# VITA-Group/UVC

Measured on AMD Instinct MI355X. Metric: images/sec UVC Stage-1 step, DeiT-Tiny budget=0.5, higher is better.
Workload: dtype bf16; 1 GPU; deit_tiny_patch16_224 Stage-1 UVC-train step, budget 0.5, per-GPU batch 512, 224x224x3 synthetic, soft distillation alpha 0.1, block gating on; global_batch=512, parallelism=dp1

## Files before the change

### include/uvc_kernels.h

```cpp
#ifndef UVC_KERNELS_H
#define UVC_KERNELS_H
#include <stdint.h>
#ifdef __cplusplus
extern "C" {
#endif

enum { UVC_F32 = 0, UVC_BF16 = 1 };

enum {
  UVC_EPI_NONE = 0,
  UVC_EPI_BIAS = 1,
  UVC_EPI_BIAS_GELU = 2,
  UVC_EPI_BIAS_RESID = 3,
  UVC_EPI_BIAS_RESID_GATE = 4,
  UVC_EPI_DGELU = 5,
  UVC_EPI_BIAS_GELU_OUT = 6,
  UVC_EPI_BIAS_GELU_GRAD = 7,
  UVC_EPI_MUL_AUX = 8,
  UVC_EPI_BIAS_GELU_GRAD_Q8 = 9,
  UVC_EPI_MUL_AUX_Q8 = 10
};
#define UVC_Q8_LO (-0.13f)
#define UVC_Q8_STEP (1.26f / 255.0f)

// ... 41 lines not shown
  void* o;
  float* lse;
  const void* dout;
  void* dqkv;
  float* delta;
  int32_t B, N, H, head_dim, dtype;
  float scale;
  const int32_t* head_keep;
  int32_t variant;
  int32_t grid;
  int32_t v_dim;
} uvc_attn_args;
int uvc_attention_fwd(const uvc_attn_args* args, void* stream);
int uvc_attention_bwd(const uvc_attn_args* args, void* stream);
int uvc_attention_bwd_vdim(const uvc_attn_args* args, void* stream);

typedef struct uvc_qkv_attn_args {
  const void* h;
  const void* w;
  const float* bias;
  void* qkv;
  void* o;
  float* lse;
  int32_t B, N, H, D, dtype;
  float scale;
  int32_t grid;
} uvc_qkv_attn_args;
int uvc_qkv_attention_supported(int32_t B, int32_t N, int32_t H, int32_t D, int32_t dtype);
int uvc_qkv_attention_fwd(const uvc_qkv_attn_args* args, void* stream);

typedef struct uvc_attn_tok_args {
  const void* qkv;
  void* o;
  const void* dout;
  void* dqkv;
  int32_t B, N, H, head_dim, ntok, dtype;
  float scale;
  const int32_t* head_keep;
} uvc_attn_tok_args;
int uvc_attention_tok_fwd(const uvc_attn_tok_args* args, void* stream);
int uvc_attention_tok_bwd(const uvc_attn_tok_args* args, void* stream);

int uvc_copy_row_groups(const void* src, void* dst, int64_t groups, int64_t group_bytes, int64_t src_group_stride, int64_t dst_group_stride,
                        void* stream);

typedef struct uvc_ln_args {
  const void* x;
  const float* gamma; const float* beta;
  void* y; float* mean; float* rstd;
  const void* dy;
  void* dx;
  const void* add1; const float* a1;
  const void* add2; const float* a2;
  float* partial;
  float* dgamma; float* dbeta;
  float* dots;
  float eps, beta_acc;
  int32_t rows, D, rows_per_group, dtype, y_is_f32, dy_is_f32;
  int64_t group_stride;
  int32_t g_lowp;
  int32_t defer_reduce;
  int32_t x_lowp;
  int32_t reserved;
} uvc_ln_args;
typedef struct uvc_ln_reduce_item { const float* partial; float* dgamma; float* dbeta; float* dots; int32_t nblocks; int32_t reserved; } uvc_ln_reduce_item;
int uvc_layernorm_bwd_reduce_batch(const uvc_ln_reduce_item* items, int32_t n, int32_t D, float beta_acc, void* stream);
int uvc_layernorm_fwd(const uvc_ln_args* args, void* stream);
int uvc_layernorm_bwd(const uvc_ln_args* args, void* stream);
int uvc_layernorm_bwd_blocks(int32_t rows);
int uvc_layernorm_bwd_nblocks(int32_t rows);

typedef struct uvc_gemm_lnbwd_args {
  const void* A; const void* W;
  const void* x; const float* mean; const float* rstd; const float* gamma;
  const void* add1; const float* a1; const void* add2; const float* a2;
  void* dx; float* partial;
  int32_t M, D, K, dtype;
  int32_t variant;
  int32_t x_lowp;
} uvc_gemm_lnbwd_args;
int uvc_gemm_lnbwd_supported(int32_t M, int32_t D, int32_t K, int32_t dtype);
int uvc_gemm_lnbwd_nblocks(int32_t M);
int uvc_gemm_nt_lnbwd(const uvc_gemm_lnbwd_args* args, void* stream);

typedef struct uvc_mlp_args {
  const void* x; const float* gamma; const float* beta;
  const void* w1; const float* b1; const void* w2; const float* b2;
  void* out;
  int32_t M, D, F;
  float eps;
  const void* x_prev; const float* gate;
  void* h; float* mean; float* rstd; void* gp; void* u;
  const float* next_gamma; const float* next_beta; void* next_h; float* next_mean; float* next_rstd;
  int32_t rows_lowp;
  int32_t reserved;
} uvc_mlp_args;
int uvc_mlp_fused_supported(int32_t D, int32_t F, int32_t dtype);
int uvc_mlp_fused_fwd(const uvc_mlp_args* args, void* stream);

typedef struct uvc_loss_args {
  const float* o; const float* o_kd; const float* y_soft; const float* teacher;
  float* loss; float* d_o; float* d_okd; float* row_scratch;
  float alpha, tau;
  int32_t B, C, kind;
} uvc_loss_args;
int uvc_distill_loss(const uvc_loss_args* args, void* stream);

int uvc_grad_sqnorm(const float* g, int64_t n, float* partial , float* sq , int32_t accumulate, void* stream);
typedef struct uvc_adamw_args {
  float* p; const float* g; float* m; float* v;
  void* p_shadow;
  const float* sq;
  float* gnorm_out;
  int64_t n;
  float lr, beta1, beta2, eps, weight_decay, max_norm;
  int32_t step;
  const uint8_t* flags;
} uvc_adamw_args;
int uvc_adamw_step(const uvc_adamw_args* args, void* stream);
int uvc_scale_by_clip(float* g, int64_t n, const float* sq, float max_norm, void* stream);

int uvc_patchify(const float* x, void* out, int32_t B, int32_t C, int32_t S, int32_t P, int32_t dtype, void* stream);
int uvc_assemble_tokens(const float* pe, const float* cls, const float* dist, const float* pos, const float* row_mask,
                        void* tok, int32_t B, int32_t P, int32_t D, int32_t ntok, int32_t tok_lowp , void* stream);
int uvc_assemble_tokens_bwd(const void* dtok, const float* pe, const float* row_mask, void* dpe, float* dpos, float* dcls,
                            float* ddist, float* dmask, int32_t B, int32_t P, int32_t D, int32_t ntok, int32_t dtype,
                            int32_t dpe_is_f32, int32_t dtok_lowp, float beta_acc, void* stream);
int uvc_colsum(const void* X, int32_t M, int32_t N, int32_t ldx, int32_t dtype, int32_t x_is_f32, float* partial, float* out,
               float alpha, const float* alpha_ptr, float beta, const float* row_weight , void* stream);
int uvc_patch_gate_sigmoid(const float* pg, float* mask, int32_t B, int32_t P, int32_t hard, void* stream);
int uvc_patch_gate_sigmoid_bwd(const float* pg, const float* dmask, float* dpg, int32_t B, int32_t P, float beta_acc, void* stream);
int uvc_patch_scores(const float* pe, const float* w, const float* bias, float* scores, int32_t rows, int32_t D, void* stream);
int uvc_patch_topk_mask(const float* scores, const float* e, float* mask, float* ysoft, float* psoft, int32_t B, int32_t P, int32_t k,
                        float tau, void* stream);
int uvc_patch_topk_mask_bwd(const float* dmask, const float* ysoft, const float* psoft, float* dscores, int32_t B, int32_t P, float tau,
                            void* stream);
int uvc_add_outer(void* X, const float* row_weight, const float* w, int32_t rows, int32_t D, int32_t dtype, int32_t x_is_f32, void* stream);
int uvc_colsum_blocks(int32_t M);
int uvc_mixup_batch(float* x, int32_t B, int32_t C, int32_t H, int32_t W, float lam, float one_minus_lam, int32_t use_cutmix,
                    int32_t yl, int32_t yh, int32_t xl, int32_t xh, void* stream);
int uvc_mixup_target(const int64_t* labels, float* y, int32_t B, int32_t C, float lam, float one_minus_lam, float on_value,
                     float off_value, void* stream);
int uvc_mlp_gather_shadows(const float* W1, const float* b1, const float* W2, const int32_t* idx, int32_t D, int32_t F, int32_t width,
                           void* w1c, void* w1t, void* w2c, void* w2t, float* b1c, int32_t dtype, void* stream);
int uvc_mlp_scatter_grads(const float* dw1c, const float* dw2c, const float* db1c, const int32_t* inv, const float* b1, const float* db2,
                          int32_t D, int32_t F, int32_t width, float* dW1, float* dW2, float* db1, float beta_acc, int32_t dtype, void* stream);
int uvc_apply_masks(float* params, const float* mask, int64_t n, void* stream);
int uvc_cast_transpose(const float* W, int32_t R, int32_t C, void* w_bf16, void* wt, int32_t dtype, void* stream);
int uvc_cast_transpose_multi(const float* params, void* shadow, int32_t n, const int64_t* srcs, const int32_t* Rs, const int32_t* Cs,
                             const int64_t* ws, const int64_t* wts, int32_t dtype, void* stream);
int uvc_exp_noise(float* out, int64_t n, uint64_t seed, uint64_t step, uint32_t site, void* stream);

int uvc_gate_distrib(const float* g, const float* e, float* d, int32_t L, int32_t mode, float eps, void* stream);
int uvc_gate_grad(const float* g, const float* d, const float* dots, float* dg, int32_t L, int32_t mode, float eps,
                  float beta_acc, void* stream);

#ifdef __cplusplus
}
#endif
#endif
```

### include/uvc_vit.h

```cpp
#ifndef UVC_VIT_H
#define UVC_VIT_H
#include <stdint.h>
#ifdef __cplusplus
extern "C" {
#endif

#define UVC_VIT_MAX_DEPTH 32

typedef struct uvc_vit_cfg {
  int32_t img_size, patch_size, in_chans, num_classes, embed_dim, depth, num_heads, hidden;
  int32_t ntok;
  int32_t dtype;
  float ln_eps;
  int32_t no_qkv_bias;
  int32_t resid_f32;
  int32_t reserved;
} uvc_vit_cfg;

typedef struct uvc_vit_offsets {
  int64_t cls_token, dist_token, pos_embed, patch_w, patch_b;
  int64_t blk[UVC_VIT_MAX_DEPTH][12];
  int64_t norm_w, norm_b, head_w, head_b, headd_w, headd_b;
  int64_t n_main;
  int64_t gate;
  int64_t gumbel_w, gumbel_b;
  int64_t patch_gating;
  int64_t skip[UVC_VIT_MAX_DEPTH][2];
  int64_t n_total;
} uvc_vit_offsets;

typedef struct uvc_vit_shadow_offsets {
  int64_t patch_w;
  int64_t blk_w[UVC_VIT_MAX_DEPTH][4];
  int64_t blk_wt[UVC_VIT_MAX_DEPTH][4];
  int64_t head_w, head_wt, headd_w, headd_wt;
  int64_t n_total;
} uvc_vit_shadow_offsets;

int uvc_vit_layout(const uvc_vit_cfg* cfg, uvc_vit_offsets* off, uvc_vit_shadow_offsets* soff);
int64_t uvc_vit_workspace_bytes(const uvc_vit_cfg* cfg, int32_t batch, int32_t training);
int uvc_stream_create(int32_t priority_class, void** out);
int uvc_vit_ws_offsets(const uvc_vit_cfg* cfg, int32_t batch, int32_t training, int64_t* pe_off, int64_t* dpe_off);

int uvc_vit_update_shadows(const uvc_vit_cfg* cfg, const float* params, void* shadow, void* stream);

typedef struct uvc_mlp_compact {
  int32_t width; int32_t reserved;
  const void* w1; const void* w1t; const void* w2; const void* w2t; const float* b1;
  float* dw1; float* dw2; float* db1;
  const int32_t* inv;
} uvc_mlp_compact;

typedef struct uvc_vit_io {
  const float* params;
  void* shadow;
  float* grads;
  void* workspace; int64_t workspace_bytes;
  const float* x;
  float* logits;
  float* logits_dist;
  const float* d_logits;
  const float* d_logits_dist;
  const float* gate_d;
  const int32_t* run_block;
  const float* patch_mask;
  float* d_patch_mask;
  int32_t batch;
  int32_t training;
  int32_t gate_mode;
  float gate_eps;
  float accumulate;
  int32_t stage_begin, stage_end;
  void* side_stream;
  const uvc_mlp_compact* mlp_compact;
  const int32_t* head_keep;
  int32_t full_tail;
  int32_t fused_train_mlp;
  const void* patches_in;
  int32_t fuse_next_ln;
  int32_t force_generic;
  int32_t head_keep_bwd;
  int32_t shared_bwd_streams;
  int32_t gelu_grad_bf16;
} uvc_vit_io;

int uvc_vit_forward(const uvc_vit_cfg* cfg, const uvc_vit_io* io, void* stream);
int uvc_vit_backward(const uvc_vit_cfg* cfg, const uvc_vit_io* io, void* stream);

typedef struct uvc_compact_block { int32_t heads, v_dim, hidden, reserved; } uvc_compact_block;
int uvc_vit_compact_layout(const uvc_vit_cfg* cfg, const uvc_compact_block* blocks, int32_t nblocks, uvc_vit_offsets* off,
                           uvc_vit_shadow_offsets* soff);
int64_t uvc_vit_compact_workspace_bytes(const uvc_vit_cfg* cfg, const uvc_compact_block* blocks, int32_t nblocks, int32_t batch);
int uvc_vit_compact_update_shadows(const uvc_vit_cfg* cfg, const uvc_compact_block* blocks, int32_t nblocks, const float* params, void* shadow,
                                   void* stream);
int uvc_vit_compact_forward(const uvc_vit_cfg* cfg, const uvc_compact_block* blocks, int32_t nblocks, const uvc_vit_io* io, void* stream);

int uvc_vit_compact_train_layout(const uvc_vit_cfg* cfg, const uvc_compact_block* blocks, int32_t nblocks, uvc_vit_offsets* off,
                                 uvc_vit_shadow_offsets* soff);
int64_t uvc_vit_compact_train_workspace_bytes(const uvc_vit_cfg* cfg, const uvc_compact_block* blocks, int32_t nblocks, int32_t batch);
int uvc_vit_compact_train_update_shadows(const uvc_vit_cfg* cfg, const uvc_compact_block* blocks, int32_t nblocks, const float* params, void* shadow,
                                         void* stream);
int uvc_vit_compact_frozen_ranges(const uvc_vit_cfg* cfg, const uvc_compact_block* blocks, int32_t nblocks, int64_t* ranges, int32_t cap,
                                  int32_t* count);
int uvc_vit_compact_train_forward(const uvc_vit_cfg* cfg, const uvc_compact_block* blocks, int32_t nblocks, const uvc_vit_io* io, void* stream);
int uvc_vit_compact_backward(const uvc_vit_cfg* cfg, const uvc_compact_block* blocks, int32_t nblocks, const uvc_vit_io* io, void* stream);

#ifdef __cplusplus
}
#endif
#endif
```

### uvc_amd/_lib.py

```python
from __future__ import annotations

import ctypes as C
import os

import torch

_HERE = os.path.dirname(os.path.abspath(__file__))
LIB_PATH = os.path.join(_HERE, "libuvc_hip.so")


class UvcHipError(RuntimeError):
    pass


class uvc_dims(C.Structure):
    _fields_ = [("L", C.c_int32), ("H", C.c_int32), ("hd", C.c_int32), ("D", C.c_int32), ("F", C.c_int32)]


class uvc_hyper(C.Structure):
    _fields_ = [(n, C.c_float) for n in ("budget", "slr", "rlr", "glr", "ylr", "plr", "zlr", "sl2wd", "z_grad_clip",
                                         "gating_weight", "eps")] + \
               [(n, C.c_int32) for n in ("gating_interval", "use_gumbel", "enable_block_gating")]


class uvc_state(C.Structure):
    _fields_ = [("s", C.c_void_p), ("r", C.c_void_p), ("y", C.c_void_p), ("p", C.c_void_p), ("z", C.c_void_p),
                ("gate", C.c_void_p), ("gate_grad", C.c_void_p), ("gate_momentum", C.c_void_p),
                ("gate_gsum", C.c_void_p), ("gate_counters", C.c_void_p), ("total_macs", C.c_void_p),
                ("embed_macs", C.c_float), ("resource_ub", C.c_float),
                ("scores1", C.c_void_p), ("scores2", C.c_void_p), ("scores3", C.c_void_p),
                ("rank1", C.c_void_p), ("rankh", C.c_void_p), ("rank3", C.c_void_p), ("out", C.c_void_p)]


class uvc_gemm_nt_args(C.Structure):
    _fields_ = [(n, C.c_void_p) for n in ("A", "B", "C", "C2", "bias", "R", "R2", "aux", "gate", "alpha_ptr")] + \
               [("alpha", C.c_float)] + \
               [(n, C.c_int32) for n in ("M", "N", "K", "lda", "ldb", "ldc", "ldr", "ldaux", "dtype", "a_is_f32",
                                         "c_is_f32", "epilogue", "force_generic", "r_is_f32")] + \
               [("ln_eps", C.c_float)] + [(n, C.c_void_p) for n in ("ln_gamma", "ln_beta", "ln_out", "ln_mean", "ln_rstd")]


class uvc_gemm_tn_args(C.Structure):
    _fields_ = [("A", C.c_void_p), ("B", C.c_void_p), ("C", C.c_void_p), ("workspace", C.c_void_p),
                ("workspace_bytes", C.c_int64), ("alpha_ptr", C.c_void_p), ("colsum_out", C.c_void_p), ("alpha", C.c_float),
                ("beta", C.c_float)] + \
               [(n, C.c_int32) for n in ("M", "N1", "N2", "lda", "ldb", "ldc", "dtype", "a_is_f32", "variant")]


class uvc_attn_args(C.Structure):
    _fields_ = [(n, C.c_void_p) for n in ("qkv", "o", "lse", "dout", "dqkv", "delta")] + \
               [(n, C.c_int32) for n in ("B", "N", "H", "head_dim", "dtype")] + [("scale", C.c_float), ("head_keep", C.c_void_p),
                                                                                ("variant", C.c_int32), ("grid", C.c_int32),
                                                                                ("v_dim", C.c_int32)]


class uvc_compact_block(C.Structure):
    _fields_ = [(n, C.c_int32) for n in ("heads", "v_dim", "hidden", "reserved")]


class uvc_qkv_attn_args(C.Structure):
    _fields_ = [(n, C.c_void_p) for n in ("h", "w", "bias", "qkv", "o", "lse")] + \
               [(n, C.c_int32) for n in ("B", "N", "H", "D", "dtype")] + [("scale", C.c_float), ("grid", C.c_int32)]


class uvc_attn_tok_args(C.Structure):
    _fields_ = [(n, C.c_void_p) for n in ("qkv", "o", "dout", "dqkv")] + \
               [(n, C.c_int32) for n in ("B", "N", "H", "head_dim", "ntok", "dtype")] + [("scale", C.c_float), ("head_keep", C.c_void_p)]


class uvc_ln_reduce_item(C.Structure):
    _fields_ = [(n, C.c_void_p) for n in ("partial", "dgamma", "dbeta", "dots")] + [("nblocks", C.c_int32), ("reserved", C.c_int32)]


class uvc_ln_args(C.Structure):
    _fields_ = [(n, C.c_void_p) for n in ("x", "gamma", "beta", "y", "mean", "rstd", "dy", "dx", "add1", "a1", "add2",
                                          "a2", "partial", "dgamma", "dbeta", "dots")] + \
               [("eps", C.c_float), ("beta_acc", C.c_float)] + \
               [(n, C.c_int32) for n in ("rows", "D", "rows_per_group", "dtype", "y_is_f32", "dy_is_f32")] + \
               [("group_stride", C.c_int64), ("g_lowp", C.c_int32), ("defer_reduce", C.c_int32), ("x_lowp", C.c_int32), ("reserved", C.c_int32)]


class uvc_gemm_lnbwd_args(C.Structure):
    _fields_ = [(n, C.c_void_p) for n in ("A", "W", "x", "mean", "rstd", "gamma", "add1", "a1", "add2", "a2", "dx", "partial")] + \
               [(n, C.c_int32) for n in ("M", "D", "K", "dtype", "variant", "x_lowp")]


class uvc_mlp_args(C.Structure):
    _fields_ = [(n, C.c_void_p) for n in ("x", "gamma", "beta", "w1", "b1", "w2", "b2", "out")] + \
               [(n, C.c_int32) for n in ("M", "D", "F")] + [("eps", C.c_float)] + \
               [(n, C.c_void_p) for n in ("x_prev", "gate", "h", "mean", "rstd", "gp", "u",
                                          "next_gamma", "next_beta", "next_h", "next_mean", "next_rstd")] + \
               [("rows_lowp", C.c_int32), ("reserved", C.c_int32)]


class uvc_loss_args(C.Structure):
    _fields_ = [(n, C.c_void_p) for n in ("o", "o_kd", "y_soft", "teacher", "loss", "d_o", "d_okd", "row_scratch")] + \
               [("alpha", C.c_float), ("tau", C.c_float), ("B", C.c_int32), ("C", C.c_int32), ("kind", C.c_int32)]


class uvc_adamw_args(C.Structure):
    _fields_ = [(n, C.c_void_p) for n in ("p", "g", "m", "v", "p_shadow", "sq", "gnorm_out")] + [("n", C.c_int64)] + \
               [(n, C.c_float) for n in ("lr", "beta1", "beta2", "eps", "weight_decay", "max_norm")] + \
               [("step", C.c_int32), ("flags", C.c_void_p)]


class uvc_unfold_args(C.Structure):
    _fields_ = [("src", C.c_void_p)] + [(n, C.c_int64) for n in ("sb", "sc", "sh", "sw")] + \
               [(n, C.c_int32) for n in ("B", "C", "H", "W", "k", "s", "p", "ldo", "out_is_f32", "dtype")] + \
               [("gamma", C.c_void_p), ("beta", C.c_void_p), ("eps", C.c_float), ("out", C.c_void_p), ("mean", C.c_void_p),
                ("rstd", C.c_void_p), ("dy", C.c_void_p), ("dy_is_f32", C.c_int32), ("dxu", C.c_void_p), ("partial", C.c_void_p),
                ("dgamma", C.c_void_p), ("dbeta", C.c_void_p), ("beta_acc", C.c_float), ("dxu_tap_major", C.c_int32)]


class uvc_t2t_stage(C.Structure):
    _fields_ = [("src", C.c_void_p)] + [(n, C.c_int64) for n in ("sb", "sc", "sh", "sw")] + \
               [(n, C.c_int32) for n in ("B", "C", "H", "W", "k", "s", "p", "T", "dim", "dimp", "dtype", "training")] + \
               [("eps", C.c_float), ("beta", C.c_float), ("need_dx", C.c_int32), ("reserved", C.c_int32)] + \
               [(n, C.c_void_p) for n in ("norm1_w", "norm1_b", "kqv_b", "w", "proj_b", "norm2_w", "norm2_b", "fc1_b", "fc2_b",
                                          "g_norm1_w", "g_norm1_b", "g_kqv_w", "g_kqv_b", "g_proj_w", "g_proj_b", "g_norm2_w", "g_norm2_b", "g_fc1_w", "g_fc1_b",
                                          "g_fc2_w", "g_fc2_b",
                                          "kqv_w", "kqv_wt", "proj_w", "proj_wt", "fc1_w", "fc1_wt", "fc2_w", "fc2_wt",
                                          "xn", "mean1", "rstd1", "kqv", "part", "kptv", "att", "x1", "h", "mean2", "rstd2", "u", "gp", "out",
                                          "dout", "da", "dh", "dx1", "datt", "dkqv", "dkptv", "dxn", "ln2_partial", "ln1_partial", "dxu", "tn_ws")] + \
               [("tn_ws_bytes", C.c_int64)]


class uvc_performer_args(C.Structure):
    _fields_ = [(n, C.c_void_p) for n in ("kqv", "w", "part", "kptv", "att")] + [("att_is_f32", C.c_int32)] + \
               [(n, C.c_void_p) for n in ("datt", "dskip", "dkqv", "dkptv")] + \
               [(n, C.c_int32) for n in ("g_is_f32", "B", "T", "dtype")]


class uvc_image_desc(C.Structure):
    _fields_ = [("src_offset", C.c_int64)] + \
               [(n, C.c_int32) for n in ("src_h", "src_w", "resize_h", "resize_w", "win_y", "win_x", "flip", "kh", "kv", "span0", "span",
                                         "order")] + [("ws_offset", C.c_int64)]


class uvc_image_prep_args(C.Structure):
    _fields_ = [("src", C.c_void_p), ("src_bytes", C.c_int64), ("desc", C.c_void_p), ("workspace", C.c_void_p),
                ("workspace_bytes", C.c_int64), ("out", C.c_void_p), ("mean", C.c_float * 3), ("std", C.c_float * 3)] + \
               [(n, C.c_int32) for n in ("B", "S", "out_dtype", "filter")]


class uvc_image_crop_desc(C.Structure):
    _fields_ = [("src_offset", C.c_int64)] + \
               [(n, C.c_int32) for n in ("img_h", "img_w", "crop_y", "crop_x", "crop_h", "crop_w", "resize_h", "resize_w", "win_y", "win_x", "flip",
                                         "kh", "kv", "span0", "span", "order")] + [("ws_offset", C.c_int64)]


class uvc_image_prep_crops_args(C.Structure):
    _fields_ = uvc_image_prep_args._fields_


UVC_F32, UVC_BF16 = 0, 1
UVC_IMAGE_OUT_F32, UVC_IMAGE_OUT_U8 = 0, 1
UVC_IMAGE_FILTER_BILINEAR, UVC_IMAGE_FILTER_BICUBIC = 0, 1
EPI_NONE, EPI_BIAS, EPI_BIAS_GELU, EPI_BIAS_RESID, EPI_BIAS_RESID_GATE, EPI_DGELU, EPI_BIAS_GELU_OUT, EPI_BIAS_GELU_GRAD, EPI_MUL_AUX = range(9)
EPI_BIAS_GELU_GRAD_Q8, EPI_MUL_AUX_Q8 = 9, 10
Q8_LO, Q8_STEP = -0.13, 1.26 / 255.0

_lib = None
VP = C.c_void_p
I32, I64, F32 = C.c_int32, C.c_int64, C.c_float

_SIGNATURES = {
    "uvc_scores": [VP, VP, uvc_dims, VP, VP, VP, VP, VP],
    "uvc_rank": [VP, VP, VP, uvc_dims, VP, VP, VP, VP],
    "uvc_prox": [VP, VP, uvc_dims, VP, VP, VP, VP, VP, VP, VP, C.c_double, VP, VP, VP, VP, VP],
    "uvc_dual_step": [C.POINTER(uvc_state), uvc_dims, uvc_hyper, VP, VP, C.c_int32, C.c_int32, VP],
    "uvc_resource": [C.POINTER(uvc_state), uvc_dims, uvc_hyper, VP, C.c_int32, VP, VP],
    "uvc_write_masks": [VP, VP, VP, uvc_dims, VP, VP, VP, VP, VP, VP],
    "uvc_gemm_nt": [C.POINTER(uvc_gemm_nt_args), VP],
    "uvc_gemm_nt_ln_supported": [I32, I32, I32, I32, I32],
    "uvc_gemm_nt_q8_supported": [I32, I32, I32, I32],
    "uvc_gemm_tn": [C.POINTER(uvc_gemm_tn_args), VP],
    "uvc_gemm_tn_workspace_bytes": [I32, I32, I32, C.POINTER(I64), C.POINTER(I32)],
    "uvc_attention_fwd": [C.POINTER(uvc_attn_args), VP],
    "uvc_attention_bwd": [C.POINTER(uvc_attn_args), VP],
    "uvc_attention_bwd_vdim": [C.POINTER(uvc_attn_args), VP],
    "uvc_qkv_attention_supported": [I32, I32, I32, I32, I32],
    "uvc_qkv_attention_fwd": [C.POINTER(uvc_qkv_attn_args), VP],
    "uvc_attention_tok_fwd": [C.POINTER(uvc_attn_tok_args), VP],
    "uvc_attention_tok_bwd": [C.POINTER(uvc_attn_tok_args), VP],
    "uvc_copy_row_groups": [VP, VP, I64, I64, I64, I64, VP],
    "uvc_layernorm_fwd": [C.POINTER(uvc_ln_args), VP],
    "uvc_layernorm_bwd": [C.POINTER(uvc_ln_args), VP],
    "uvc_layernorm_bwd_blocks": [I32],
    "uvc_layernorm_bwd_nblocks": [I32],
    "uvc_layernorm_bwd_reduce_batch": [C.POINTER(uvc_ln_reduce_item), I32, I32, F32, VP],
    "uvc_gemm_lnbwd_supported": [I32, I32, I32, I32],
    "uvc_gemm_lnbwd_nblocks": [I32],
    "uvc_gemm_nt_lnbwd": [C.POINTER(uvc_gemm_lnbwd_args), VP],
    "uvc_distill_loss": [C.POINTER(uvc_loss_args), VP],
    "uvc_grad_sqnorm": [VP, I64, VP, VP, I32, VP],
    "uvc_adamw_step": [C.POINTER(uvc_adamw_args), VP],
    "uvc_scale_by_clip": [VP, I64, VP, F32, VP],
    "uvc_patchify": [VP, VP, I32, I32, I32, I32, I32, VP],
    "uvc_assemble_tokens": [VP, VP, VP, VP, VP, VP, I32, I32, I32, I32, I32, VP],
    "uvc_assemble_tokens_bwd": [VP, VP, VP, VP, VP, VP, VP, VP, I32, I32, I32, I32, I32, I32, I32, F32, VP],
    "uvc_colsum": [VP, I32, I32, I32, I32, I32, VP, VP, F32, VP, F32, VP, VP],
    "uvc_patch_gate_sigmoid": [VP, VP, I32, I32, I32, VP],
    "uvc_patch_gate_sigmoid_bwd": [VP, VP, VP, I32, I32, F32, VP],
    "uvc_patch_scores": [VP, VP, VP, VP, I32, I32, VP],
    "uvc_patch_topk_mask": [VP, VP, VP, VP, VP, I32, I32, I32, F32, VP],
    "uvc_patch_topk_mask_bwd": [VP, VP, VP, VP, I32, I32, F32, VP],
    "uvc_add_outer": [VP, VP, VP, I32, I32, I32, I32, VP],
    "uvc_colsum_blocks": [I32],
    "uvc_apply_masks": [VP, VP, I64, VP],
    "uvc_mlp_gather_shadows": [VP, VP, VP, VP, I32, I32, I32, VP, VP, VP, VP, VP, I32, VP],
    "uvc_mlp_scatter_grads": [VP, VP, VP, VP, VP, VP, I32, I32, I32, VP, VP, VP, F32, I32, VP],
    "uvc_mixup_batch": [VP, I32, I32, I32, I32, F32, F32, I32, I32, I32, I32, I32, VP],
    "uvc_mixup_target": [VP, VP, I32, I32, F32, F32, F32, F32, VP],
    "uvc_stream_create": [I32, C.POINTER(VP)],
    "uvc_mlp_fused_supported": [I32, I32, I32],
    "uvc_mlp_fused_fwd": [C.POINTER(uvc_mlp_args), VP],
    "uvc_cast_transpose": [VP, I32, I32, VP, VP, I32, VP],
    "uvc_cast_transpose_multi": [VP, VP, I32, VP, VP, VP, VP, VP, I32, VP],
    "uvc_exp_noise": [VP, I64, C.c_uint64, C.c_uint64, C.c_uint32, VP],
    "uvc_gate_distrib": [VP, VP, VP, I32, I32, F32, VP],
    "uvc_gate_grad": [VP, VP, VP, VP, I32, I32, F32, F32, VP],
    "uvc_image_prep_workspace": [VP, I32, I32, I64, C.POINTER(I64)],
    "uvc_image_prep_workspace_filter": [VP, I32, I32, I64, I32, C.POINTER(I64)],
    "uvc_image_prep": [C.POINTER(uvc_image_prep_args), VP],
    "uvc_image_prep_crops_workspace": [VP, I32, I32, I64, C.POINTER(I64)],
    "uvc_image_prep_crops_workspace_filter": [VP, I32, I32, I64, I32, C.POINTER(I64)],
    "uvc_image_prep_crops": [C.POINTER(uvc_image_prep_crops_args), VP],
    "uvc_unfold_ln_fwd": [C.POINTER(uvc_unfold_args), VP],
    "uvc_unfold_ln_bwd": [C.POINTER(uvc_unfold_args), VP],
    "uvc_unfold_bwd_blocks": [I32],
    "uvc_fold_tokens": [VP, I32, I32, I32, VP, I32, I32, I32, I32, I32, I32, I32, I32, I32, VP],
    "uvc_performer_splits": [I32, I32],
    "uvc_performer_fwd": [C.POINTER(uvc_performer_args), VP],
    "uvc_performer_bwd": [C.POINTER(uvc_performer_args), VP],
    "uvc_t2t_stage_forward": [C.POINTER(uvc_t2t_stage), VP],
    "uvc_t2t_stage_backward": [C.POINTER(uvc_t2t_stage), VP],
}


VIT_SYMBOLS = ["uvc_vit_layout", "uvc_vit_workspace_bytes", "uvc_vit_ws_offsets", "uvc_vit_update_shadows", "uvc_vit_forward",
               "uvc_vit_backward", "uvc_vit_compact_layout", "uvc_vit_compact_workspace_bytes", "uvc_vit_compact_update_shadows",
               "uvc_vit_compact_forward",
               "uvc_vit_compact_train_layout", "uvc_vit_compact_train_workspace_bytes", "uvc_vit_compact_train_update_shadows",
               "uvc_vit_compact_frozen_ranges", "uvc_vit_compact_train_forward", "uvc_vit_compact_backward"]


def side_stream(device, priority_class=None):
    import torch
    if priority_class is None:
        priority_class = int(os.environ.get("UVC_SIDE_PRIORITY", "0"))
    out = VP()
    with torch.cuda.device(device):
        check(lib().uvc_stream_create(priority_class, C.byref(out)), "uvc_stream_create")
    return torch.cuda.ExternalStream(out.value, device=device)


def exported_symbols():
    return list(_SIGNATURES) + ["uvc_last_error"] + VIT_SYMBOLS


def lib():
    global _lib
    if _lib is None:
        if not os.path.exists(LIB_PATH):
            raise UvcHipError(f"{LIB_PATH} not found: build it with `python -m uvc_amd.build` "
                              "(there is no CPU fallback for the product path)")
        _lib = C.CDLL(LIB_PATH)
        _lib.uvc_last_error.restype = C.c_char_p
        for name, args in _SIGNATURES.items():
            fn = getattr(_lib, name)
            fn.argtypes = args
            fn.restype = C.c_int
    return _lib


def check(rc: int, what: str):
# ... 17 lines not shown
```

### uvc_amd/csrc/gemm.hip

```cpp
#include <type_traits>
#include "common.h"
#include "../../include/uvc_kernels.h"

template <typename T> struct Mma;
template <> struct Mma<bf16_t> {
  static constexpr int CH = 8;
  static constexpr int KSTEP = 32;
  typedef bf16x8 Frag;
  static __device__ __forceinline__ f32x4 mma(const Frag& a, const Frag& b, f32x4 c) {
    return __builtin_amdgcn_mfma_f32_16x16x32_bf16(a, b, c, 0, 0, 0);
  }
};
template <> struct Mma<float> {
  static constexpr int CH = 4;
  static constexpr int KSTEP = 16;
  typedef f32x4 Frag;
  static __device__ __forceinline__ f32x4 mma(const Frag& a, const Frag& b, f32x4 c) {
#pragma unroll
    for (int j = 0; j < 4; ++j) c = __builtin_amdgcn_mfma_f32_16x16x4f32(a[j], b[j], c, 0, 0, 0);
    return c;
  }
};

template <typename TS, typename T> struct ChunkLoad;
// ... 990 lines not shown
  if (q8 && (p->force_generic == 1 || p->a_is_f32 || p->c_is_f32 || p->ln_out || !uvc_gemm_nt_q8_supported(p->M, p->N, p->K, p->dtype) ||
             (p->ldaux ? p->ldaux : p->ldc) % 8 || p->ldc % 8 || p->ldb != p->K))
    return uvc_set_error_msg(UVC_ERR_UNSUPPORTED, "uvc_gemm_nt: the one-byte GELU' epilogues need bf16 A / C, K = 192, N % 256 == 0, M >= 4096 (uvc_gemm_nt_q8_supported)");
  NtArgs a;
  a.A = p->A; a.B = p->B; a.C = p->C; a.C2 = p->C2; a.bias = p->bias; a.R = p->R; a.R2 = p->R2; a.aux = p->aux;
  a.dptr = p->gate; a.M = p->M; a.N = p->N; a.K = p->K; a.lda = p->lda; a.ldb = p->ldb; a.ldc = p->ldc;
  a.ldr = p->ldr ? p->ldr : p->ldc; a.ldaux = p->ldaux ? p->ldaux : p->ldc; a.alpha = p->alpha; a.alpha_ptr = p->alpha_ptr;
  a.ln_gamma = p->ln_gamma; a.ln_beta = p->ln_beta; a.ln_out = p->ln_out; a.ln_mean = p->ln_mean; a.ln_rstd = p->ln_rstd; a.ln_eps = p->ln_eps;
  a.no_dma = p->force_generic == 2;
  const bool generic = p->force_generic == 1;
  hipStream_t st = (hipStream_t)stream;
  if (p->ln_out) {
    if (!p->ln_gamma || !p->ln_beta || (p->ln_mean != nullptr) != (p->ln_rstd != nullptr))
      return uvc_set_error_msg(UVC_ERR_ARG, "uvc_gemm_nt: ln_out needs ln_gamma, ln_beta (and ln_mean, ln_rstd together)");
    if (p->N == 384) {
      if (!uvc_gemm_nt_ln_supported(p->M, p->N, p->K, p->dtype, e) || generic || p->a_is_f32 || p->c_is_f32 || p->alpha != 1.0f || p->alpha_ptr || !row384_fwd_ok(a, e))
        return uvc_set_error_msg(UVC_ERR_UNSUPPORTED, "uvc_gemm_nt: ln_out is not available for this problem (uvc_gemm_nt_ln_supported; N = 384: bf16 C and R only)");
      return launch_row384_fwd(a, e, st);
    }
    if (!uvc_gemm_nt_ln_supported(p->M, p->N, p->K, p->dtype, e) || generic || p->a_is_f32 || p->alpha != 1.0f || p->alpha_ptr ||
        a.ldb != a.K || !wsn16_dma_ok(a) || ((uintptr_t)p->ln_out & 7) != 0)
      return uvc_set_error_msg(UVC_ERR_UNSUPPORTED, "uvc_gemm_nt: ln_out is not available for this problem (uvc_gemm_nt_ln_supported)");
    if (p->M % 16 != 0 && (p->C == (const void*)p->R || p->C == (const void*)p->R2))
      return uvc_set_error_msg(UVC_ERR_ARG, "uvc_gemm_nt: with ln_out and M % 16 != 0 the last row tile is computed twice: C must not alias R / R2");
    if (p->K == 192) return p->c_is_f32 ? launch_wsn16_dma<UVC_EPI_BIAS_RESID, 6, true, 7, false>(a, st) : launch_wsn16_dma<UVC_EPI_BIAS_RESID, 6, true, 7, true>(a, st);
    return p->c_is_f32 ? launch_wsn<float>(a, e, st) : launch_wsn<bf16_t>(a, e, st);
  }
  if (p->dtype == UVC_F32) {
    if (!p->a_is_f32 || !p->c_is_f32) return uvc_set_error_msg(UVC_ERR_ARG, "uvc_gemm_nt: float32 mode needs float32 A and C");
    return launch_nt_epi<float, float, float>(a, e, st);
  }
  if (p->dtype != UVC_BF16) return uvc_set_error_msg(UVC_ERR_ARG, "uvc_gemm_nt: dtype must be UVC_F32 or UVC_BF16");
  {
    if (!p->force_generic && !p->a_is_f32 && e == UVC_EPI_BIAS_RESID && p->K == 192 && p->N == 192 && a.ldb == 192 &&
        p->M >= 4096 && p->M % 16 == 0 && p->alpha == 1.0f && !p->alpha_ptr && wsn16_dma_ok(a))
      return p->c_is_f32 ? launch_wsn16_dma<UVC_EPI_BIAS_RESID, 6, false, 7, false>(a, st) : launch_wsn16_dma<UVC_EPI_BIAS_RESID, 6, false, 7, true>(a, st);
  }
  const bool ws = !generic && ws_ok(a, p->c_is_f32 ? 4 : 8);
  if (q8 && !ws) return uvc_set_error_msg(UVC_ERR_UNSUPPORTED, "uvc_gemm_nt: the one-byte GELU' epilogues exist in the K = 192 streaming kernel only");
  if (!generic && ws384_ok(a, e, p->c_is_f32 ? 4 : 8, p->a_is_f32 != 0)) {
    if (!p->c_is_f32 && a.N % 128 == 0 && a.N >= 512 && p->force_generic != 5) return launch_ws384<bf16_t, 8>(a, e, st);
    return p->c_is_f32 ? launch_ws384<float>(a, e, st) : launch_ws384<bf16_t>(a, e, st);
  }
  if (!generic && wsn_ok(a, e, p->a_is_f32 != 0))
    return p->c_is_f32 ? launch_wsn<float>(a, e, st) : launch_wsn<bf16_t>(a, e, st);
  if ((p->force_generic >> 8) == 1) {
    if (!nt8p_takes(a, p->a_is_f32 != 0)) return uvc_set_error_msg(UVC_ERR_UNSUPPORTED, "uvc_gemm_nt: shape not taken by the 8-phase kernel");
    return p->c_is_f32 ? launch_nt8p_f32(a, e, p->force_generic & 255, st) : launch_nt8p_bf16(a, e, p->force_generic & 255, st);
  }
  const bool few_tiles_wide = !p->c_is_f32 && a.N % 256 == 0 && nt8p_takes(a, p->a_is_f32 != 0);
  if (!generic && !a.no_dma && !(p->force_generic == 3 && few_tiles_wide && a.N < 1792) &&
      nt256_takes(a, p->a_is_f32 != 0, p->force_generic == 3 || p->force_generic == 4))
    return p->c_is_f32 ? launch_nt256_f32(a, e, st) : launch_nt256_bf16(a, e, st);
  if (!generic && !a.no_dma && few_tiles_wide && (a.M >= 2048 || p->force_generic == 3))
    return launch_nt8p_bf16(a, e, 0, st);
  if (p->a_is_f32) {
    if ((p->lda % 8) != 0) return uvc_set_error_msg(UVC_ERR_ARG, "uvc_gemm_nt: lda");
    if (ws) return p->c_is_f32 ? launch_ws<float, float>(a, e, st) : launch_ws<float, bf16_t>(a, e, st);
    return p->c_is_f32 ? launch_nt_epi<float, bf16_t, float>(a, e, st) : launch_nt_epi<float, bf16_t, bf16_t>(a, e, st);
  }
  if (ws) return p->c_is_f32 ? launch_ws<bf16_t, float>(a, e, st) : launch_ws<bf16_t, bf16_t>(a, e, st);
  return p->c_is_f32 ? launch_nt_epi<bf16_t, bf16_t, float>(a, e, st) : launch_nt_epi<bf16_t, bf16_t, bf16_t>(a, e, st);
}

template <typename T> struct Raw4L;
template <> struct Raw4L<float> {
  typedef f32x4 V;
  static __device__ __forceinline__ V ld(const float* p) { return *reinterpret_cast<const f32x4*>(p); }
  static __device__ __forceinline__ V zero() { return f32x4{0.f, 0.f, 0.f, 0.f}; }
  static __device__ __forceinline__ f32x4 cvt(const V& r) { return r; }
};
template <> struct Raw4L<bf16_t> {
  typedef u32x2 V;
  static __device__ __forceinline__ V ld(const bf16_t* p) { return *reinterpret_cast<const u32x2*>(p); }
  static __device__ __forceinline__ V zero() { return u32x2{0u, 0u}; }
  static __device__ __forceinline__ f32x4 cvt(const V& r) {
    return f32x4{__uint_as_float(r[0] << 16), __uint_as_float(r[0] & 0xffff0000u), __uint_as_float(r[1] << 16), __uint_as_float(r[1] & 0xffff0000u)};
  }
};
struct LnbArgs {
  const void* A; const void* W; const void* x; const float* mean; const float* rstd; const float* gamma;
  const void* add1; const float* a1; const void* add2; const float* a2; void* dx; float* partial;
  int M, K, want_dots;
};

template <int KT, bool XLOW>
__global__ __launch_bounds__(768) void k_gemm_wsn_lnbwd(LnbArgs g) {
  typedef Resid<typename std::conditional<XLOW, bf16_t, float>::type> XS_;
  typedef bf16_t T;
  typedef Mma<T> MM;
  constexpr int K = KT * 32, NTH = 768, D = 192, NWV = 12;
  constexpr int ROWB = K * 2 + 32, CPR = K / 8;
  constexpr int NLD = (16 * CPR + NTH - 1) / NTH;
  extern __shared__ __attribute__((aligned(16))) char smem[];
  char* sA0 = smem;
  char* sA1 = smem + 16 * ROWB;
  float* sRed = reinterpret_cast<float*>(smem + 2 * 16 * ROWB);
  float* sGam = sRed + 2 * 16 * NWV * 2;
  const int tid = threadIdx.x, lane = tid & 63, w = tid >> 6, gq = lane >> 4, li = lane & 15;
  const T* __restrict__ A = reinterpret_cast<const T*>(g.A);
  const T* __restrict__ W = reinterpret_cast<const T*>(g.W);
  const T* __restrict__ add1 = reinterpret_cast<const T*>(g.add1);
  const T* __restrict__ add2 = reinterpret_cast<const T*>(g.add2);
  T* __restrict__ dx = reinterpret_cast<T*>(g.dx);
  const int ntiles = (g.M + 15) / 16;
  const int n = w * 16 + gq * 4;

  typename MM::Frag bf[KT];
#pragma unroll
  for (int ks = 0; ks < KT; ++ks)
    bf[ks] = __builtin_bit_cast(typename MM::Frag, *reinterpret_cast<const u32x4*>(W + (size_t)(w * 16 + li) * K + (ks * 4 + gq) * 8));
  if (tid < D) sGam[tid] = g.gamma[tid];
  const float a1 = g.a1 ? *g.a1 : 1.f, a2 = g.a2 ? *g.a2 : 1.f;
  f32x4 dgam = {0.f, 0.f, 0.f, 0.f}, dbet = {0.f, 0.f, 0.f, 0.f};
  float dotA = 0.f, dotB = 0.f;
  constexpr float invD = 1.0f / (float)D;

  u32x4 ra[NLD];
  unsigned aoff[NLD];
#pragma unroll
  for (int i = 0; i < NLD; ++i) { const int id = tid + NTH * i; aoff[i] = (unsigned)((id / CPR) * K + (id % CPR) * 8); }
  auto gload = [&](int tile) {
    const int m0 = tile * 16;
    const u32x4 z = {0u, 0u, 0u, 0u};
#pragma unroll
    for (int i = 0; i < NLD; ++i) {
      const int row = (tid + NTH * i) / CPR;
      ra[i] = (row < 16 && m0 + row < g.M) ? *reinterpret_cast<const u32x4*>(A + ((unsigned)(m0 * K) + aoff[i])) : z;
    }
  };
  auto lstore = [&](char* buf) {
#pragma unroll
    for (int i = 0; i < NLD; ++i) {
      const int id = tid + NTH * i, row = id / CPR, c = id % CPR;
      if (row < 16) *reinterpret_cast<u32x4*>(buf + row * ROWB + c * 16) = ra[i];
    }
  };

  int tile = blockIdx.x;
  if (tile < ntiles) {
    gload(tile);
    lstore(sA0);
  }
  __syncthreads();
  int par = 0;
  for (; tile < ntiles; tile += gridDim.x) {
    const int next = tile + gridDim.x;
    if (next < ntiles) gload(next);
    const int m = tile * 16 + li;
    const bool ok = m < g.M;
    const unsigned ro = (unsigned)(ok ? m : 0) * (unsigned)D + (unsigned)n;
    const f32x4 xv = XS_::f4(XS_::ld4(g.x, ro));
    u32x2 r1 = {0u, 0u}, r2 = {0u, 0u};
    if (add1) r1 = *reinterpret_cast<const u32x2*>(add1 + ro);
    if (add2) r2 = *reinterpret_cast<const u32x2*>(add2 + ro);
    const float mean = g.mean[ok ? m : 0], rstd = ok ? g.rstd[m] : 0.f;
    const char* buf = par ? sA1 : sA0;
    f32x4 c0 = {0.f, 0.f, 0.f, 0.f};
#pragma unroll
    for (int ks = 0; ks < KT; ++ks) {
      c0 = MM::mma(bf[ks], lds_frag<T>(buf + li * ROWB + (ks * 4 + gq) * 16), c0);
      if (KT > 18 && (ks % 6) == 5) __builtin_amdgcn_sched_barrier(0);
    }
    float* red = sRed + par * (16 * NWV * 2);
    {
      const f32x4 gam = *reinterpret_cast<const f32x4*>(sGam + n);
      float p1 = 0.f, p2 = 0.f;
#pragma unroll
      for (int e = 0; e < 4; ++e) {
        const float xh = (xv[e] - mean) * rstd;
        const float gy = c0[e] * gam[e];
        dgam[e] += c0[e] * xh;
        dbet[e] += c0[e];
        p1 += gy;
        p2 += gy * xh;
      }
      p1 = sum_rows4(p1);
      p2 = sum_rows4(p2);
      if (gq == 0) *reinterpret_cast<f32x2*>(red + (li * NWV + w) * 2) = f32x2{p1, p2};
    }
    if (next < ntiles) lstore(par ? sA0 : sA1);
    __syncthreads();
    float c1 = 0.f, c2 = 0.f;
#pragma unroll
    for (int q = 0; q < NWV / 2; ++q) {
      const f32x4 t = *reinterpret_cast<const f32x4*>(red + li * NWV * 2 + q * 4);
      c1 += t[0]; c2 += t[1]; c1 += t[2]; c2 += t[3];
    }
    c1 *= invD; c2 *= invD;
    if (ok) {
      const f32x4 gam = *reinterpret_cast<const f32x4*>(sGam + n);
      const f32x4 v1 = {__uint_as_float(r1[0] << 16), __uint_as_float(r1[0] & 0xffff0000u), __uint_as_float(r1[1] << 16), __uint_as_float(r1[1] & 0xffff0000u)};
      const f32x4 v2 = {__uint_as_float(r2[0] << 16), __uint_as_float(r2[0] & 0xffff0000u), __uint_as_float(r2[1] << 16), __uint_as_float(r2[1] & 0xffff0000u)};
      float o[4];
#pragma unroll
      for (int e = 0; e < 4; ++e) {
        const float xh = (xv[e] - mean) * rstd;
        o[e] = rstd * (c0[e] * gam[e] - c1 - xh * c2);
        if (add1) o[e] += a1 * v1[e];
        if (add2) { o[e] += a2 * v2[e]; dotB += v2[e] * xv[e]; }
        dotA += o[e] * xv[e];
      }
      u32x2 q; q[0] = pack_bf16x2(o[0], o[1]); q[1] = pack_bf16x2(o[2], o[3]);
      *reinterpret_cast<u32x2*>(dx + ro) = q;
    }
    par ^= 1;
  }
#pragma unroll
  for (int e = 0; e < 4; ++e) {
#pragma unroll
    for (int o = 1; o < 16; o <<= 1) { dgam[e] += __shfl_xor(dgam[e], o, 64); dbet[e] += __shfl_xor(dbet[e], o, 64); }
  }
  float* P = g.partial + (size_t)blockIdx.x * (2 * D + 2);
  if (li == 0) {
    *reinterpret_cast<f32x2*>(P + n) = f32x2{dgam[0], dgam[1]}; *reinterpret_cast<f32x2*>(P + n + 2) = f32x2{dgam[2], dgam[3]};
    *reinterpret_cast<f32x2*>(P + D + n) = f32x2{dbet[0], dbet[1]}; *reinterpret_cast<f32x2*>(P + D + n + 2) = f32x2{dbet[2], dbet[3]};
  }
  dotA = wave_sum(dotA); dotB = wave_sum(dotB);
  __syncthreads();
  if (lane == 0) { sRed[2 * w] = dotA; sRed[2 * w + 1] = dotB; }
  __syncthreads();
  if (tid < 2) {
    float t = 0.f;
#pragma unroll
    for (int q = 0; q < NWV; ++q) t += sRed[2 * q + tid];
    P[2 * D + tid] = t;
  }
}

__device__ __forceinline__ unsigned lds_addr(const void* p) { return (unsigned)(size_t)(LDS_PTR(char))(char*)p; }
__device__ __forceinline__ u32x4 ds_read128_asm(unsigned addr, int off) {
  u32x4 v;
  asm volatile("ds_read_b128 %0, %1 offset:%2" : "=v"(v) : "v"(addr), "n"(off));
  return v;
}
template <int OFF> __device__ __forceinline__ u32x4 ds_read128(unsigned addr) {
  u32x4 v;
  asm volatile("ds_read_b128 %0, %1 offset:%2" : "=v"(v) : "v"(addr), "n"(OFF));
  return v;
}
__device__ __forceinline__ u32x2 ds_read64_a(unsigned addr) { u32x2 v; asm volatile("ds_read_b64 %0, %1" : "=v"(v) : "v"(addr)); return v; }
__device__ __forceinline__ float ds_read32_a(unsigned addr) { float v; asm volatile("ds_read_b32 %0, %1" : "=v"(v) : "v"(addr)); return v; }
__device__ __forceinline__ void ds_write64_a(unsigned addr, f32x2 v) { asm volatile("ds_write_b64 %0, %1" ::"v"(addr), "v"(v) : "memory"); }
template <int N> __device__ __forceinline__ void wait_lgkm() { asm volatile("s_waitcnt lgkmcnt(%0)" ::"n"(N) : "memory"); }
template <int N> __device__ __forceinline__ void wait_vm() { asm volatile("s_waitcnt vmcnt(%0)" ::"n"(N) : "memory"); }
#define TIE4(a, b, c, d) asm volatile("" : "+v"(a), "+v"(b), "+v"(c), "+v"(d))

template <int KT, bool HAS2, bool XLOW>
__global__ __launch_bounds__(768) void k_gemm_wsn_lnbwd_dma(LnbArgs g) {
  typedef bf16_t T;
  typedef Mma<T> MM;
  constexpr int K = KT * 32, D = 192, NWV = 12;
  constexpr int ROWB = K * 2 + 32, SA = ROWB / 16;
  constexpr int NA = (16 * SA + 63) / 64;
  constexpr int XSZ = XLOW ? 2 : 4, XSL = D * XSZ / 16;
  constexpr int XS = XSL + 2, XB = XS * 16, NX = (16 * XS + 63) / 64;
  constexpr int PS = 26, PB = PS * 16, NP = (16 * PS + 63) / 64;
  constexpr int I_X = NA, I_1 = I_X + NX, I_2 = I_1 + NP, NI = I_2 + NP;
  constexpr int STAGE = NI * 1024;
  static_assert((16 * SA) % 64 == 32, "spare half block behind the A image");
  constexpr int MR_OFF = (NA - 1) * 1024 + 512;
  static_assert(NI <= 5 * NWV && 3 * STAGE + 2 * 16 * NWV * 8 + D * 4 <= 160 * 1024, "ring does not fit");
  extern __shared__ __attribute__((aligned(16))) char smem[];
  float* sRed = reinterpret_cast<float*>(smem + 3 * STAGE);
  const int tid = threadIdx.x, lane = tid & 63, gq = lane >> 4, li = lane & 15;
  const int w = __builtin_amdgcn_readfirstlane(tid >> 6);
  const T* __restrict__ W = reinterpret_cast<const T*>(g.W);
  T* __restrict__ dx = reinterpret_cast<T*>(g.dx);
  const int ntiles = g.M / 16;
  const int n = w * 16 + gq * 4;

  typename MM::Frag bf[KT];
#pragma unroll
  for (int ks = 0; ks < KT; ++ks)
    bf[ks] = __builtin_bit_cast(typename MM::Frag, *reinterpret_cast<const u32x4*>(W + (size_t)(w * 16 + li) * K + (ks * 4 + gq) * 8));
  float* sGam = sRed + 2 * 16 * NWV * 2;
  if (tid < D) sGam[tid] = g.gamma[tid];
  const unsigned gaddr = lds_addr(sGam) + (unsigned)n * 4u;
  const float a1 = g.a1 ? *g.a1 : 1.f, a2 = g.a2 ? *g.a2 : 1.f;
  const bool has1 = g.add1 != nullptr;
  constexpr bool has2 = HAS2;
  f32x4 dgam = {0.f, 0.f, 0.f, 0.f}, dbet = {0.f, 0.f, 0.f, 0.f};
  float dotA = 0.f, dotB = 0.f;
  constexpr float invD = 1.0f / (float)D;

  const char* rb[5]; unsigned rstride[5], rdst[5], loff[5];
#pragma unroll
  for (int q = 0; q < 5; ++q) {
    int I = q * NWV + w;
    const bool dup = I >= NI || (I >= I_1 && I < I_2 && !has1) || (I >= I_2 && !has2);
    if (dup) I = w;
    const int sl = (I - (I < I_X ? 0 : I < I_1 ? I_X : I < I_2 ? I_1 : I_2)) * 64 + lane;
    rdst[q] = (unsigned)I * 1024u;
    if (I < I_X) {
      const int row = sl / SA, c = sl % SA;
      rb[q] = reinterpret_cast<const char*>(g.A); rstride[q] = 16u * K * 2u;
      loff[q] = row < 16 ? (unsigned)(row * K * 2 + (c < K / 8 ? c : 0) * 16) : 0u;
    } else if (I < I_1) {
      const int row = sl / XS, c = sl % XS;
      rb[q] = reinterpret_cast<const char*>(g.x); rstride[q] = 16u * D * (unsigned)XSZ;
      loff[q] = row < 16 ? (unsigned)(row * D * XSZ + (c < XSL ? c : 0) * 16) : 0u;
    } else {
      const int row = sl / PS, c = sl % PS;
      rb[q] = reinterpret_cast<const char*>(I < I_2 ? g.add1 : g.add2); rstride[q] = 16u * D * 2u;
      loff[q] = row < 16 ? (unsigned)(row * D * 2 + (c < 24 ? c : 0) * 16) : 0u;
    }
  }
  const long long mr_delta = reinterpret_cast<const char*>(g.rstd) - reinterpret_cast<const char*>(g.mean);
  const unsigned mr_lo = (unsigned)(lane & 3) * 16u;
  const bool mr_lane = lane >= 32 && lane < 40, mr_r = lane >= 36;
  auto issue_q = [&](int tile, int st, int q) {
    const int t = tile < ntiles ? tile : ntiles - 1;
    if (q < 5) {
      const char* src = rb[q] + ((unsigned long long)(unsigned)t * (unsigned long long)rstride[q] + (unsigned long long)loff[q]);
      char* dst = smem + st * STAGE + rdst[q];
      __builtin_amdgcn_global_load_lds((const void __attribute__((address_space(1)))*)src, (void __attribute__((address_space(3)))*)dst, 16, 0, 0);
    } else if (mr_lane) {
      const char* src = reinterpret_cast<const char*>(g.mean) + ((unsigned long long)(unsigned)t * 64ull + mr_lo) + (mr_r ? mr_delta : 0ll);
      char* dst = smem + st * STAGE + (NA - 1) * 1024;
      __builtin_amdgcn_global_load_lds((const void __attribute__((address_space(1)))*)src, (void __attribute__((address_space(3)))*)dst, 16, 0, 0);
    }
  };
  auto issue = [&](int tile, int st) {
#pragma unroll
    for (int q = 0; q < 6; ++q) issue_q(tile, st, q);
  };
  const unsigned s0 = lds_addr(smem);
  const unsigned fragoff = (unsigned)(li * ROWB + gq * 16);
  const unsigned xoff = (unsigned)(I_X * 1024 + li * XB + n * XSZ), poff = (unsigned)(I_1 * 1024 + li * PB + n * 2), moff = (unsigned)(MR_OFF + li * 4);
  const unsigned redr = lds_addr(sRed) + (unsigned)(li * NWV * 8);

  int tile = blockIdx.x;
  issue(tile, 0);
  issue(tile + gridDim.x, 1);
  wait_vm<6>();
  __builtin_amdgcn_s_barrier();
  int st = 0, par = 0;
  for (; tile < ntiles; tile += gridDim.x) {
    const int nt_ = tile + 2 * (int)gridDim.x, ns_ = st == 0 ? 2 : st - 1;
    const unsigned sb = s0 + (unsigned)(st * STAGE);
    f32x4 c0 = {0.f, 0.f, 0.f, 0.f};
    constexpr bool DB = KT <= 18;
    u32x4 fa[2], fb[2];
    const unsigned fr = sb + fragoff;
#define RD2(dst, ks0) dst[0] = ds_read128<(ks0) * 64>(fr); dst[1] = ds_read128<(ks0) * 64 + 64>(fr);
#define GROUP(gk, cur, nxt) if ((gk) < KT / 2) { \
      if (DB) { if ((gk) + 1 < KT / 2) { RD2(nxt, ((gk) + 1) * 2) wait_lgkm<2>(); } else wait_lgkm<0>(); \
                asm volatile("" : "+v"(cur[0]), "+v"(cur[1])); \
                c0 = MM::mma(bf[(gk) * 2], __builtin_bit_cast(typename MM::Frag, cur[0]), c0); \
                c0 = MM::mma(bf[(gk) * 2 + 1], __builtin_bit_cast(typename MM::Frag, cur[1]), c0); } \
      else if (((gk) & 1) == 0) { RD2(fa, (gk) * 2) RD2(fb, (gk) * 2 + 2) wait_lgkm<0>();  \
             asm volatile("" : "+v"(fa[0]), "+v"(fa[1]), "+v"(fb[0]), "+v"(fb[1])); \
             c0 = MM::mma(bf[(gk) * 2], __builtin_bit_cast(typename MM::Frag, fa[0]), c0); \
             c0 = MM::mma(bf[(gk) * 2 + 1], __builtin_bit_cast(typename MM::Frag, fa[1]), c0); \
             c0 = MM::mma(bf[(gk) * 2 + 2], __builtin_bit_cast(typename MM::Frag, fb[0]), c0); \
             c0 = MM::mma(bf[(gk) * 2 + 3], __builtin_bit_cast(typename MM::Frag, fb[1]), c0); } }
    static_assert(KT % 2 == 0 && KT <= 24, "pairs of k-steps");
    if (DB) { RD2(fa, 0) }
    GROUP(0, fa, fb) issue_q(nt_, ns_, 0); GROUP(1, fb, fa) GROUP(2, fa, fb) issue_q(nt_, ns_, 1); GROUP(3, fb, fa)
    GROUP(4, fa, fb) issue_q(nt_, ns_, 2); GROUP(5, fb, fa) GROUP(6, fa, fb) issue_q(nt_, ns_, 3); GROUP(7, fb, fa)
    GROUP(8, fa, fb) issue_q(nt_, ns_, 4); issue_q(nt_, ns_, 5); GROUP(9, fb, fa) GROUP(10, fa, fb) GROUP(11, fb, fa)
#undef GROUP
#undef RD2
    typename Resid<typename std::conditional<XLOW, bf16_t, float>::type>::Raw4 xr;
    if constexpr (XLOW) asm volatile("ds_read_b64 %0, %1" : "=v"(xr) : "v"(sb + xoff));
    else xr = ds_read128<0>(sb + xoff);
    u32x2 r1 = {0u, 0u}, r2 = {0u, 0u};
    if (has1) asm volatile("ds_read_b64 %0, %1" : "=v"(r1) : "v"(sb + poff));
    if (has2) asm volatile("ds_read_b64 %0, %1 offset:%2" : "=v"(r2) : "v"(sb + poff), "n"((I_2 - I_1) * 1024));
    float mean, rstd;
    asm volatile("ds_read_b32 %0, %1" : "=v"(mean) : "v"(sb + moff));
    asm volatile("ds_read_b32 %0, %1 offset:64" : "=v"(rstd) : "v"(sb + moff));
    u32x4 gr = ds_read128<0>(gaddr);
    wait_lgkm<0>();
    asm volatile("" : "+v"(xr), "+v"(r1), "+v"(r2), "+v"(mean), "+v"(rstd), "+v"(gr));
    const f32x4 xv = Resid<typename std::conditional<XLOW, bf16_t, float>::type>::f4(xr);
    f32x4 gam = __builtin_bit_cast(f32x4, gr);
    {
      float p1 = 0.f, p2 = 0.f;
#pragma unroll
      for (int e = 0; e < 4; ++e) {
        const float xh = (xv[e] - mean) * rstd;
        const float gy = c0[e] * gam[e];
        dgam[e] += c0[e] * xh;
        dbet[e] += c0[e];
        p1 += gy;
        p2 += gy * xh;
      }
      p1 = sum_rows4(p1);
      p2 = sum_rows4(p2);
      if (gq == 0) ds_write64_a(redr + (unsigned)(par * 16 * NWV * 8 + w * 8), f32x2{p1, p2});
#pragma unroll
      for (int e = 0; e < 4; ++e) c0[e] *= gam[e];
    }
    wait_vm<6>();
    wait_lgkm<0>();
    __builtin_amdgcn_s_barrier();
    float c1 = 0.f, c2 = 0.f;
    {
      const unsigned rr = redr + (unsigned)(par * 16 * NWV * 8);
      u32x4 t0 = ds_read128<0>(rr), t1 = ds_read128<16>(rr), t2 = ds_read128<32>(rr);
      wait_lgkm<0>();
      asm volatile("" : "+v"(t0), "+v"(t1), "+v"(t2));
      {
        const f32x4 a = __builtin_bit_cast(f32x4, t0), b = __builtin_bit_cast(f32x4, t1), c = __builtin_bit_cast(f32x4, t2);
        c1 += a[0]; c2 += a[1]; c1 += a[2]; c2 += a[3]; c1 += b[0]; c2 += b[1]; c1 += b[2]; c2 += b[3]; c1 += c[0]; c2 += c[1]; c1 += c[2]; c2 += c[3];
      }
      t0 = ds_read128<48>(rr); t1 = ds_read128<64>(rr); t2 = ds_read128<80>(rr);
      wait_lgkm<0>();
      asm volatile("" : "+v"(t0), "+v"(t1), "+v"(t2));
      {
        const f32x4 a = __builtin_bit_cast(f32x4, t0), b = __builtin_bit_cast(f32x4, t1), c = __builtin_bit_cast(f32x4, t2);
        c1 += a[0]; c2 += a[1]; c1 += a[2]; c2 += a[3]; c1 += b[0]; c2 += b[1]; c1 += b[2]; c2 += b[3]; c1 += c[0]; c2 += c[1]; c1 += c[2]; c2 += c[3];
      }
    }
    c1 *= invD; c2 *= invD;
    {
      const f32x4 v1 = {__uint_as_float(r1[0] << 16), __uint_as_float(r1[0] & 0xffff0000u), __uint_as_float(r1[1] << 16), __uint_as_float(r1[1] & 0xffff0000u)};
      const f32x4 v2 = {__uint_as_float(r2[0] << 16), __uint_as_float(r2[0] & 0xffff0000u), __uint_as_float(r2[1] << 16), __uint_as_float(r2[1] & 0xffff0000u)};
      float o[4];
#pragma unroll
      for (int e = 0; e < 4; ++e) {
        const float xh = (xv[e] - mean) * rstd;
        o[e] = rstd * (c0[e] - c1 - xh * c2);
        if (has1) o[e] += a1 * v1[e];
        if (has2) { o[e] += a2 * v2[e]; dotB += v2[e] * xv[e]; }
        dotA += o[e] * xv[e];
      }
      u32x2 q; q[0] = pack_bf16x2(o[0], o[1]); q[1] = pack_bf16x2(o[2], o[3]);
      *reinterpret_cast<u32x2*>(dx + ((size_t)(tile * 16 + li) * D + n)) = q;
    }
    st = st == 2 ? 0 : st + 1;
    par ^= 1;
  }
  wait_vm<0>();
  __syncthreads();
#pragma unroll
  for (int e = 0; e < 4; ++e) {
#pragma unroll
    for (int o = 1; o < 16; o <<= 1) { dgam[e] += __shfl_xor(dgam[e], o, 64); dbet[e] += __shfl_xor(dbet[e], o, 64); }
  }
  float* P = g.partial + (size_t)blockIdx.x * (2 * D + 2);
  if (li == 0) {
    *reinterpret_cast<f32x2*>(P + n) = f32x2{dgam[0], dgam[1]}; *reinterpret_cast<f32x2*>(P + n + 2) = f32x2{dgam[2], dgam[3]};
    *reinterpret_cast<f32x2*>(P + D + n) = f32x2{dbet[0], dbet[1]}; *reinterpret_cast<f32x2*>(P + D + n + 2) = f32x2{dbet[2], dbet[3]};
  }
  dotA = wave_sum(dotA); dotB = wave_sum(dotB);
  if (lane == 0) { sRed[2 * w] = dotA; sRed[2 * w + 1] = dotB; }
  __syncthreads();
  if (tid < 2) {
    float t = 0.f;
#pragma unroll
    for (int q = 0; q < NWV; ++q) t += sRed[2 * q + tid];
    P[2 * D + tid] = t;
  }
}
#undef TIE4

template <int EPI, int KT, bool LN, int NST, bool RLOW>
__global__ __launch_bounds__(768) void k_gemm_wsn16_dma(NtArgs g) {
  typedef bf16_t T;
  typedef Mma<T> MM;
  constexpr int K = KT * 32, D = 192, NWV = 12;
  constexpr int ROWB = K * 2 + 32, SA = ROWB / 16;
  constexpr int NA = (16 * SA + 63) / 64;
  constexpr int RSZ = RLOW ? 2 : 4, RSL = D * RSZ / 16;
  constexpr int XS = RSL + 2, XB = XS * 16, NX = (16 * XS + 63) / 64;
  constexpr bool GATE = EPI == UVC_EPI_BIAS_RESID_GATE;
  constexpr int I_R = NA, I_R2 = I_R + NX, NI = I_R2 + (GATE ? NX : 0);
  constexpr int STAGE = NI * 1024;
  constexpr int NPW = (NI + NWV - 1) / NWV;
  constexpr int LN_BYTES = LN ? 2 * 16 * NWV * 8 + 3 * D * 4 : 0;
  static_assert(NST >= 3 && NPW <= 5 && NST * STAGE + LN_BYTES <= 160 * 1024, "ring does not fit");
  extern __shared__ __attribute__((aligned(16))) char smem[];
  const int tid = threadIdx.x, lane = tid & 63, gq = lane >> 4, li = lane & 15;
  const int w = __builtin_amdgcn_readfirstlane(tid >> 6);
  const T* __restrict__ W = reinterpret_cast<const T*>(g.B);
  char* __restrict__ C = reinterpret_cast<char*>(g.C);
  const int ntiles = (g.M + 15) / 16;
  const int n = w * 16 + gq * 4;
  float* const sRed = reinterpret_cast<float*>(smem + NST * STAGE);
  float* const sGB = sRed + 2 * 16 * NWV * 2;
  if (LN) {
    if (tid < D) { sGB[tid] = g.ln_gamma[tid]; sGB[D + tid] = g.ln_beta[tid]; sGB[2 * D + tid] = g.bias[tid]; }
  }
  const unsigned gaddr = lds_addr(sGB) + (unsigned)n * 4u;
  const unsigned redr = lds_addr(sRed) + (unsigned)(li * NWV * 8);
  typename MM::Frag bf[KT];
#pragma unroll
  for (int ks = 0; ks < KT; ++ks)
    bf[ks] = __builtin_bit_cast(typename MM::Frag, *reinterpret_cast<const u32x4*>(W + (size_t)(w * 16 + li) * K + (ks * 4 + gq) * 8));
  float alpha = g.alpha;
  if (g.alpha_ptr) alpha *= *g.alpha_ptr;
  float d0 = 0.f, d1 = 1.f;
  if (GATE) { d0 = g.dptr[0]; d1 = g.dptr[1]; }
  f32x4 bias4 = {0.f, 0.f, 0.f, 0.f};
  if (!LN) bias4 = *reinterpret_cast<const f32x4*>(g.bias + n);

  const char* rb[NPW]; unsigned rstride[NPW], rdst[NPW], loff[NPW];
#pragma unroll
  for (int q = 0; q < NPW; ++q) {
    int I = q * NWV + w;
    if (I >= NI) I = w;
    const int sl = (I - (I < I_R ? 0 : I < I_R2 ? I_R : I_R2)) * 64 + lane;
    rdst[q] = (unsigned)I * 1024u;
    if (I < I_R) {
      const int row = sl / SA, c = sl % SA;
      rb[q] = reinterpret_cast<const char*>(g.A); rstride[q] = K * 2u;
      loff[q] = row < 16 ? (unsigned)(row * K * 2 + (c < K / 8 ? c : 0) * 16) : 0u;
    } else {
      const int row = sl / XS, c = sl % XS;
      rb[q] = reinterpret_cast<const char*>(I < I_R2 ? g.R : g.R2); rstride[q] = (unsigned)(D * RSZ);
      loff[q] = row < 16 ? (unsigned)(row * D * RSZ + (c < RSL ? c : 0) * 16) : 0u;
    }
  }
  auto issue = [&](int tile, int st) {
    const int t = tile < ntiles ? tile : ntiles - 1;
    const unsigned r0 = (unsigned)min(t * 16, g.M - 16);
#pragma unroll
    for (int q = 0; q < NPW; ++q) {
      const char* src = rb[q] + ((unsigned long long)r0 * (unsigned long long)rstride[q] + (unsigned long long)loff[q]);
      char* dst = smem + st * STAGE + rdst[q];
      __builtin_amdgcn_global_load_lds((const void __attribute__((address_space(1)))*)src, (void __attribute__((address_space(3)))*)dst, 16, 0, 0);
    }
  };
  const unsigned s0 = lds_addr(smem);
  const unsigned fragoff = (unsigned)(li * ROWB + gq * 16), roff = (unsigned)(I_R * 1024 + li * XB + n * RSZ);

// ... 96 lines not shown
      __builtin_amdgcn_s_barrier();
      const f32x4 r = RS::f4(rr), r2 = RS::f4(rr2);
      float o[4];
#pragma unroll
      for (int e = 0; e < 4; ++e) {
        o[e] = epi_scale_bias(c0[e], alpha, bias4[e]);
        o[e] += r[e];
        if (GATE) o[e] = epi_gate_mix(o[e], r2[e], d0, d1);
      }
      char* cp = C + ((size_t)(min(tile * 16, g.M - 16) + li) * g.ldc + n) * RSZ;
      if constexpr (RLOW) { u32x2 q; q[0] = pack_bf16x2(o[0], o[1]); q[1] = pack_bf16x2(o[2], o[3]); *reinterpret_cast<u32x2*>(cp) = q; }
      else *reinterpret_cast<f32x4*>(cp) = f32x4{o[0], o[1], o[2], o[3]};
    } else {
      u32x4 bq = ds_read128<2 * D * 4>(gaddr);
      wait_lgkm<0>();
      asm volatile("" : "+v"(rr), "+v"(rr2), "+v"(bq));
      const f32x4 r = RS::f4(rr), r2 = RS::f4(rr2), bv = __builtin_bit_cast(f32x4, bq);
      float o[4];
#pragma unroll
      for (int e = 0; e < 4; ++e) {
        o[e] = epi_scale_bias(c0[e], alpha, bv[e]);
        o[e] += r[e];
        if (GATE) o[e] = epi_gate_mix(o[e], r2[e], d0, d1);
      }
      u32x2 oq = {0u, 0u};
      if constexpr (RLOW) {
        oq[0] = pack_bf16x2(o[0], o[1]); oq[1] = pack_bf16x2(o[2], o[3]);
        const f32x4 t = Resid<bf16_t>::f4(oq);
#pragma unroll
        for (int e = 0; e < 4; ++e) o[e] = t[e];
      }
      {
        const float sm = sum_rows4((o[0] + o[1]) + (o[2] + o[3]));
        const float mw = sm * (1.0f / 16.0f);
        float qw = 0.f;
#pragma unroll
        for (int e = 0; e < 4; ++e) { const float dd = o[e] - mw; qw += dd * dd; }
        qw = sum_rows4(qw);
        if (gq == 0) ds_write64_a(redr + (unsigned)(par * 16 * NWV * 8 + w * 8), f32x2{mw, qw});
      }
      prow0 = min(tile * 16, g.M - 16);
      if constexpr (RLOW) *reinterpret_cast<u32x2*>(C + (size_t)prow0 * g.ldc * RSZ + (unsigned)((li * g.ldc + n) * RSZ)) = oq;
      else *reinterpret_cast<f32x4*>(C + (size_t)prow0 * g.ldc * RSZ + (unsigned)((li * g.ldc + n) * RSZ)) = f32x4{o[0], o[1], o[2], o[3]};
#pragma unroll
      for (int e = 0; e < 4; ++e) po[e] = o[e];
      have_prev = true;
      wait_vm<(NST - 2) * NPW>();
      wait_lgkm<0>();
      __builtin_amdgcn_s_barrier();
      par ^= 1;
    }
    st = st == NST - 1 ? 0 : st + 1;
  }
  if (LN && have_prev) {
    ln_issue(std::integral_constant<int, 0>{});
    wait_lgkm<0>(); ln_first();
    ln_issue(std::integral_constant<int, 32>{});
    wait_lgkm<0>(); ln_acc();
    ln_issue(std::integral_constant<int, 64>{}); lgr = ds_read128<0>(gaddr); lbr = ds_read128<D * 4>(gaddr);
    wait_lgkm<0>(); ln_acc(); ln_finish();
  }
  wait_vm<0>();
}

int launch_row384_lnbwd(const LnbArgs& a, int x_lowp, hipStream_t st);

extern "C" int uvc_gemm_lnbwd_supported(int32_t M, int32_t D, int32_t K, int32_t dtype) {
  if (dtype != UVC_BF16 || M < 4096) return 0;
  if (D == 192) return K == 768 || K == 576;
  return D == 384 && K % 64 == 0 && K >= 128 && (int64_t)M * K < (1ll << 30);
}
extern "C" int uvc_gemm_lnbwd_nblocks(int32_t M) { const int nt = ceil_div(M, 16); return nt < 256 ? nt : 256; }

extern "C" int uvc_gemm_nt_lnbwd(const uvc_gemm_lnbwd_args* p, void* stream) {
  if (!p || !p->A || !p->W || !p->x || !p->mean || !p->rstd || !p->gamma || !p->dx || !p->partial)
    return uvc_set_error_msg(UVC_ERR_ARG, "uvc_gemm_nt_lnbwd: null pointer");
  if (!uvc_gemm_lnbwd_supported(p->M, p->D, p->K, p->dtype))
    return uvc_set_error_msg(UVC_ERR_UNSUPPORTED, "uvc_gemm_nt_lnbwd: bf16, M >= 4096, D = 192 with K in {576, 768} or D = 384 with K % 64 == 0");
  if ((((uintptr_t)p->A | (uintptr_t)p->W | (uintptr_t)p->x | (uintptr_t)p->gamma) & 15) != 0 ||
      (((uintptr_t)p->add1 | (uintptr_t)p->add2 | (uintptr_t)p->dx | (uintptr_t)p->partial) & 7) != 0)
    return uvc_set_error_msg(UVC_ERR_ARG, "uvc_gemm_nt_lnbwd: misaligned buffer");
  LnbArgs a;
  a.A = p->A; a.W = p->W; a.x = p->x; a.mean = p->mean; a.rstd = p->rstd; a.gamma = p->gamma; a.add1 = p->add1; a.a1 = p->a1;
  a.add2 = p->add2; a.a2 = p->a2; a.dx = p->dx; a.partial = p->partial; a.M = p->M; a.K = p->K; a.want_dots = 1;
  const int grid = uvc_gemm_lnbwd_nblocks(p->M);
  hipStream_t st = (hipStream_t)stream;
  if (p->D == 384) return launch_row384_lnbwd(a, p->x_lowp, st);
#define LNB_LAUNCH(KT_) { \
    const size_t sh = (size_t)2 * 16 * (KT_ * 64 + 32) + (2 * 16 * 12 * 2 + 192) * sizeof(float); \
    if (p->x_lowp) { UVC_MAX_LDS(sh, k_gemm_wsn_lnbwd<KT_, true>); k_gemm_wsn_lnbwd<KT_, true><<<grid, 768, sh, st>>>(a); } \
    else { UVC_MAX_LDS(sh, k_gemm_wsn_lnbwd<KT_, false>); k_gemm_wsn_lnbwd<KT_, false><<<grid, 768, sh, st>>>(a); } }
  const bool use_dma = p->variant != 1;
  const bool al16 = (((uintptr_t)p->add1 | (uintptr_t)p->add2 | (uintptr_t)p->mean | (uintptr_t)p->rstd) & 15) == 0;
#define LNB_DMA_ONE(KT_, H2_, XL_) { UVC_MAX_LDS(sh, k_gemm_wsn_lnbwd_dma<KT_, H2_, XL_>); k_gemm_wsn_lnbwd_dma<KT_, H2_, XL_><<<grid, 768, sh, st>>>(a); }
#define LNB_LAUNCH_DMA(KT_) { \
    constexpr int NA_ = (16 * (KT_ * 4 + 2) + 63) / 64; \
    const int NI_ = NA_ + (p->x_lowp ? 7 : 13) + 7 + 7; \
    const size_t sh = (size_t)3 * NI_ * 1024 + (2 * 16 * 12 * 2 + 192) * sizeof(float); \
    if (p->x_lowp) { if (p->add2) LNB_DMA_ONE(KT_, true, true) else LNB_DMA_ONE(KT_, false, true) } \
    else { if (p->add2) LNB_DMA_ONE(KT_, true, false) else LNB_DMA_ONE(KT_, false, false) } }
  if (use_dma && al16 && p->M % 16 == 0) { if (p->K == 768) LNB_LAUNCH_DMA(24) else LNB_LAUNCH_DMA(18) }
  else if (p->K == 768) LNB_LAUNCH(24) else LNB_LAUNCH(18)
#undef LNB_LAUNCH_DMA
#undef LNB_DMA_ONE
#undef LNB_LAUNCH
  UVC_CHECK_LAUNCH();
  return UVC_OK;
}

#define NT_EPILOGUE_TILE(NH, MROW0, NCOL0, PD1, PD2)                                                                                 \
  {                                                                                                                           \
    constexpr bool PRE_ = sizeof(TC) == 2 && EpiOperands<EPI>::COUNT > 0;                                                     \
    constexpr int PD_ = EpiOperands<EPI>::COUNT >= 2 ? (PD2) : (PD1);                                                              \
    EpiPre<2> pre_[PD_];                                                                                                      \
    if constexpr (PRE_) {                                                                                                     \
      _Pragma("unroll") for (int h = 0; h < PD_ && h < (NH); ++h) nt_epilogue_prefetch<EPI, 16>(g, lane, (MROW0) + h * 16, (NCOL0), pre_[h]); \
    }                                                                                                                         \
    _Pragma("unroll") for (int h = 0; h < (NH); ++h) {                                                                        \
      _Pragma("unroll") for (int j = 0; j < 4; ++j)                                                                           \
        *reinterpret_cast<f32x4*>(stg_at<true>(stg, lane & 15, j * 4 + (lane >> 4))) = acc[h][j];                            \
      __builtin_amdgcn_wave_barrier();                                                                                        \
      nt_epilogue_rows<T, TC, EPI, 16, true, PRE_>(g, stg, lane, (MROW0) + h * 16, (NCOL0), alpha, d0, d1, bias_v, &pre_[h % PD_]); \
      if constexpr (PRE_) { if (h + PD_ < (NH)) nt_epilogue_prefetch<EPI, 16>(g, lane, (MROW0) + (h + PD_) * 16, (NCOL0), pre_[h % PD_]); } \
      __builtin_amdgcn_wave_barrier();                                                                                        \
    }                                                                                                                         \
  }

constexpr int G2_BM = 256, G2_BN = 256, G2_BK = 64;
constexpr int G2_OPB = 256 * 128;
constexpr int G2_STAGE = 2 * G2_OPB;
constexpr int G2_EPI = 8 * 16 * 64 * 4;
constexpr int G2_LDS = 2 * G2_STAGE + G2_EPI;

struct G2Frags { u32x4 a[8]; u32x4 b[4]; };

__device__ __forceinline__ bool g2_tile(int v, int tiles_m, int tiles_n, int& bm, int& bn) {
  const int xcd = v & 7, q = v >> 3;
  bn = q % tiles_n; bm = (q / tiles_n) * 8 + xcd;
  return bm < tiles_m;
}

template <typename TC, int EPI>
__global__ __launch_bounds__(512, 2) void k_gemm_nt256(NtArgs g, int tiles_m, int tiles_n, int nvirt) {
  typedef bf16_t T;
  typedef Mma<T> MM;
  extern __shared__ __attribute__((aligned(16))) char smem[];
  const int tid = threadIdx.x, lane = tid & 63;
  const int w = __builtin_amdgcn_readfirstlane(tid >> 6);
  const int wm = w >> 2, wn = w & 3;

  const __amdgpu_buffer_rsrc_t rA = __builtin_amdgcn_make_buffer_rsrc(const_cast<void*>(g.A), 0, (int)(((size_t)(g.M - 1) * g.lda + g.K) * 2), 0x00020000);
  const __amdgpu_buffer_rsrc_t rB = __builtin_amdgcn_make_buffer_rsrc(const_cast<void*>(g.B), 0, (int)(((size_t)(g.N - 1) * g.ldb + g.K) * 2), 0x00020000);
  const int lrow = lane >> 3, lchunk = (lane & 7) ^ lrow;
  const unsigned laneA = (unsigned)(((w * 8 + lrow) * g.lda + lchunk * 8) * 2), laneB = (unsigned)(((w * 8 + lrow) * g.ldb + lchunk * 8) * 2);
  const unsigned stepA = (unsigned)(64 * g.lda * 2), stepB = (unsigned)(64 * g.ldb * 2);
  auto issue1 = [&](int t, unsigned voA, unsigned voB, int kt, int st) {
    char* base = smem + st * G2_STAGE + w * 1024;
    const unsigned kb = (unsigned)(kt * G2_BK * 2);
    if (t < 4) __builtin_amdgcn_raw_ptr_buffer_load_lds(rA, (__attribute__((address_space(3))) void*)(base + t * 8192), 16, laneA + (voA + kb + t * stepA), 0, 0, 0);
    else __builtin_amdgcn_raw_ptr_buffer_load_lds(rB, (__attribute__((address_space(3))) void*)(base + G2_OPB + (t - 4) * 8192), 16, laneB + (voB + kb + (t - 4) * stepB), 0, 0, 0);
  };
  const unsigned s0 = lds_addr(smem);
  const unsigned sw0 = (unsigned)((((lane >> 4)) ^ (lane & 7)) * 16);
  const unsigned fa0 = s0 + (unsigned)((wm * 128 + (lane & 15)) * 128) + sw0;
  const unsigned fb0 = s0 + (unsigned)(G2_OPB + (wn * 64 + (lane & 15)) * 128) + sw0;
  auto rdfrags = [&](G2Frags& F, int st, int ks) {
    const unsigned a = (fa0 ^ (unsigned)(ks * 64)) + (unsigned)(st * G2_STAGE), b = (fb0 ^ (unsigned)(ks * 64)) + (unsigned)(st * G2_STAGE);
    F.b[0] = ds_read128<0 * 2048>(b); F.b[1] = ds_read128<1 * 2048>(b); F.b[2] = ds_read128<2 * 2048>(b); F.b[3] = ds_read128<3 * 2048>(b);
    F.a[0] = ds_read128<0 * 2048>(a); F.a[1] = ds_read128<1 * 2048>(a); F.a[2] = ds_read128<2 * 2048>(a); F.a[3] = ds_read128<3 * 2048>(a);
    F.a[4] = ds_read128<4 * 2048>(a); F.a[5] = ds_read128<5 * 2048>(a); F.a[6] = ds_read128<6 * 2048>(a); F.a[7] = ds_read128<7 * 2048>(a);
  };
  auto tie = [&](G2Frags& F) {
    asm volatile("" : "+v"(F.a[0]), "+v"(F.a[1]), "+v"(F.a[2]), "+v"(F.a[3]), "+v"(F.a[4]), "+v"(F.a[5]), "+v"(F.a[6]), "+v"(F.a[7]),
                      "+v"(F.b[0]), "+v"(F.b[1]), "+v"(F.b[2]), "+v"(F.b[3]));
  };
  f32x4 acc[8][4];
  auto mfma_row = [&](const G2Frags& F, int i) {
#pragma unroll
    for (int j = 0; j < 4; ++j) acc[i][j] = MM::mma(__builtin_bit_cast(typename MM::Frag, F.b[j]), __builtin_bit_cast(typename MM::Frag, F.a[i]), acc[i][j]);
  };
  float alpha = g.alpha;
  if (g.alpha_ptr) alpha *= *g.alpha_ptr;
  float d0 = 0.f, d1 = 1.f;
  if (EPI == UVC_EPI_BIAS_RESID_GATE) { d0 = g.dptr[0]; d1 = g.dptr[1]; }
  float* const stg = reinterpret_cast<float*>(smem + 2 * G2_STAGE) + w * (16 * 64);

  const int nk = g.K / G2_BK;
  int v = blockIdx.x, bm = 0, bn = 0;
// ... 1418 lines not shown
```

### uvc_amd/csrc/vit_engine.hip

```cpp
#include "engine_host.h"

namespace {

int check_cfg(const uvc_vit_cfg* c) {
  if (!c) return uvc_set_error_msg(UVC_ERR_ARG, "uvc_vit: null cfg");
  if (c->depth <= 0 || c->depth > UVC_VIT_MAX_DEPTH) return uvc_set_error_msg(UVC_ERR_ARG, "uvc_vit: depth out of range");
  if (c->embed_dim != c->num_heads * 64) return uvc_set_error_msg(UVC_ERR_UNSUPPORTED, "uvc_vit: head_dim must be 64");
  if (c->embed_dim % 64 || c->hidden % 64 || c->embed_dim > 1024) return uvc_set_error_msg(UVC_ERR_UNSUPPORTED, "uvc_vit: embed_dim/hidden must be multiples of 64, embed_dim <= 1024");
  if (c->img_size % c->patch_size || c->patch_size % 4) return uvc_set_error_msg(UVC_ERR_ARG, "uvc_vit: img_size/patch_size");
  if (c->ntok != 1 && c->ntok != 2) return uvc_set_error_msg(UVC_ERR_ARG, "uvc_vit: ntok must be 1 or 2");
  if (c->dtype != UVC_F32 && c->dtype != UVC_BF16) return uvc_set_error_msg(UVC_ERR_ARG, "uvc_vit: dtype");
  if (c->num_classes <= 0 || c->num_classes % 8) return uvc_set_error_msg(UVC_ERR_UNSUPPORTED, "uvc_vit: num_classes must be a positive multiple of 8");
  const int np = (c->img_size / c->patch_size) * (c->img_size / c->patch_size);
  if (np > 1024) return uvc_set_error_msg(UVC_ERR_UNSUPPORTED, "uvc_vit: more than 1024 patches (the attention kernels take N <= 1026)");
  return UVC_OK;
}

struct BlockBufs {
  void* x; void* h1; void* qkv; void* o; float* lse; float* mean1; float* rstd1;
  void* x1; void* h2; float* mean2; float* rstd2; void* a; void* u;
};
struct TailBufs {
  void* xc; void* oc; void* x1c; void* h2c; float* mean2c; float* rstd2c; void* ac; void* uc; void* xoutc;
  void* gAc; void* dAc; void* dHc; void* gBc; void* dOc;
// ... 106 lines not shown
int flush_tn(Ctx& c) {
  if (!c.side || c.n_pend == 0) return UVC_OK;
  hipError_t e = hipEventRecord(g_ev_raw, (hipStream_t)c.st);
  if (e == hipSuccess) e = hipStreamWaitEvent((hipStream_t)c.side, g_ev_raw, 0);
  if (e != hipSuccess) return uvc_set_error(e, __FILE__, __LINE__);
  for (int i = 0; i < c.n_pend; ++i) { if (int r = launch_tn(c, c.pend[i], c.side)) return r; }
  c.n_pend = 0;
  return UVC_OK;
}
int join_side(Ctx& c) {
  if (!c.side) return UVC_OK;
  if (int r = flush_tn(c)) return r;
  hipError_t e = hipEventRecord(g_ev_join, (hipStream_t)c.side);
  if (e == hipSuccess) e = hipStreamWaitEvent((hipStream_t)c.st, g_ev_join, 0);
  if (e != hipSuccess) return uvc_set_error(e, __FILE__, __LINE__);
  return UVC_OK;
}

const void* sh(const Ctx& c, int64_t off) { return (const char*)c.io->shadow + off * c.d.tsz; }
const void* wmat(const Ctx& c, int64_t poff, int64_t soff) { return c.d.dtype == UVC_F32 ? (const void*)(c.io->params + poff) : sh(c, soff); }

struct NextLn { const float* gamma; const float* beta; void* h; float* mean; float* rstd; };
int nt(const Ctx& c, const void* A, int a_f32, const void* B, void* C, int c_f32, int M, int N, int K, int epi, const float* bias = nullptr,
       const void* R = nullptr, const void* R2 = nullptr, const void* aux = nullptr, const float* gate = nullptr, void* C2 = nullptr,
       const float* alpha_ptr = nullptr, int lda = 0, int ldc = 0, const NextLn* ln = nullptr) {
  uvc_gemm_nt_args a;
  memset(&a, 0, sizeof(a));
  if (ln) { a.ln_gamma = ln->gamma; a.ln_beta = ln->beta; a.ln_out = ln->h; a.ln_mean = ln->mean; a.ln_rstd = ln->rstd; a.ln_eps = c.d.eps; }
  a.A = A; a.B = B; a.C = C; a.C2 = C2; a.bias = bias; a.R = R; a.R2 = R2; a.aux = aux; a.gate = gate; a.alpha_ptr = alpha_ptr;
  a.alpha = 1.0f; a.M = M; a.N = N; a.K = K; a.lda = lda ? lda : K; a.ldb = K; a.ldc = ldc ? ldc : N; a.ldr = a.ldc; a.ldaux = a.ldc;
  a.dtype = c.d.dtype; a.a_is_f32 = a_f32 || c.d.dtype == UVC_F32; a.c_is_f32 = c_f32 || c.d.dtype == UVC_F32; a.epilogue = epi;
  a.r_is_f32 = a.c_is_f32;
  a.force_generic = ln ? 0 : c.io->force_generic;
  return uvc_gemm_nt(&a, c.st);
}
int launch_tn(Ctx& c, const Ctx::PendingTn& t, void* stream) {
  uvc_gemm_tn_args a;
  memset(&a, 0, sizeof(a));
  a.colsum_out = t.bias_grad;
  a.A = t.A; a.B = t.B; a.C = t.C; a.workspace = (c.side && stream == c.st) ? c.w.tn_ws_main : c.w.tn_ws; a.workspace_bytes = c.w.tn_ws_bytes; a.alpha_ptr = t.alpha_ptr; a.alpha = 1.0f;
  a.beta = t.scratch ? 0.f : c.io->accumulate; a.M = t.M; a.N1 = t.N1; a.N2 = t.N2; a.lda = t.lda ? t.lda : t.N1; a.ldb = t.ldb ? t.ldb : t.N2; a.ldc = t.N2;
  a.dtype = c.d.dtype; a.a_is_f32 = t.a_f32 || c.d.dtype == UVC_F32;
  return uvc_gemm_tn(&a, stream);
}
int tn(Ctx& c, const void* A, int a_f32, const void* B, float* C, float* bias_grad, int M, int N1, int N2, const float* alpha_ptr = nullptr,
       int lda = 0, int ldb = 0, bool scratch = false) {
  const Ctx::PendingTn t = {A, a_f32, B, C, bias_grad, M, N1, N2, alpha_ptr, lda, ldb, scratch};
  if (!c.side || c.tn_inline) return launch_tn(c, t, c.st);
  if (c.n_pend == 8) { if (int r = flush_tn(c)) return r; }
  c.pend[c.n_pend++] = t;
  return UVC_OK;
}
int csum(const Ctx& c, const void* X, int x_f32, float* out, int M, int N, const float* alpha_ptr = nullptr, int ldx = 0) {
  return uvc_colsum(X, M, N, ldx ? ldx : N, c.d.dtype, x_f32 || c.d.dtype == UVC_F32, c.w.cs_partial, out, 1.0f, alpha_ptr, c.io->accumulate, nullptr, c.st);
}
int ln_fwd(const Ctx& c, const void* x, int64_t pw, int64_t pb, void* y, float* mean, float* rstd, int rows, int rpg, int64_t gs) {
  uvc_ln_args a;
  memset(&a, 0, sizeof(a));
  a.x = x; a.x_lowp = c.d.rlow; a.gamma = c.io->params + pw; a.beta = c.io->params + pb; a.y = y; a.mean = mean; a.rstd = rstd; a.eps = c.d.eps;
  a.rows = rows; a.D = c.d.D; a.rows_per_group = rpg; a.group_stride = gs; a.dtype = c.d.dtype;
  return uvc_layernorm_fwd(&a, c.st);
}
int flush_ln(Ctx& c) {
  if (c.n_ln == 0) return UVC_OK;
  const int e = uvc_layernorm_bwd_reduce_batch(c.ln_items, c.n_ln, c.d.D, c.io->accumulate, c.st);
  c.n_ln = 0;
  return e;
}
int ln_bwd(Ctx& c, const void* dy, const void* x, int64_t pw, int64_t pb, const float* mean, const float* rstd, void* dx,
           const void* add1, const float* a1, const void* add2, const float* a2, float* dots, int rows, int rpg, int64_t gs) {
  uvc_ln_args a;
  memset(&a, 0, sizeof(a));
  a.x = x; a.x_lowp = c.d.rlow; a.gamma = c.io->params + pw; a.mean = (float*)mean; a.rstd = (float*)rstd; a.dy = dy; a.dx = dx; a.add1 = add1; a.a1 = a1;
  if (c.n_ln >= 2 * c.d.L + 1) { if (int e = flush_ln(c)) return e; }
  a.add2 = add2; a.a2 = a2; a.partial = c.w.ln_partial + c.w.ln_region * c.n_ln; a.dgamma = c.io->grads + pw; a.dbeta = c.io->grads + pb; a.dots = dots;
  a.defer_reduce = 1;
  uvc_ln_reduce_item& it = c.ln_items[c.n_ln++];
  it.partial = a.partial; it.dgamma = a.dgamma; it.dbeta = a.dbeta; it.dots = dots; it.nblocks = uvc_layernorm_bwd_nblocks(rows); it.reserved = 0;
  a.eps = c.d.eps; a.beta_acc = c.io->accumulate; a.rows = rows; a.D = c.d.D; a.rows_per_group = rpg; a.group_stride = gs; a.dtype = c.d.dtype;
  a.g_lowp = c.d.dtype == UVC_BF16;
  return uvc_layernorm_bwd(&a, c.st);
}
bool lnb_fused_ok(const Ctx& c, int K) { return c.io->force_generic != 1 && uvc_gemm_lnbwd_supported(c.d.M, c.d.D, K, c.d.dtype) != 0; }
int dgrad_ln_bwd(Ctx& c, const void* A, const void* Wt, int K, const void* x, int64_t pw, int64_t pb, const float* mean, const float* rstd, void* dx,
                 const void* add1, const float* a1, const void* add2, const float* a2, float* dots) {
  if (c.n_ln >= 2 * c.d.L + 1) { if (int e = flush_ln(c)) return e; }
  uvc_gemm_lnbwd_args a;
  memset(&a, 0, sizeof(a));
  a.A = A; a.W = Wt; a.x = x; a.mean = mean; a.rstd = rstd; a.gamma = c.io->params + pw; a.add1 = add1; a.a1 = a1; a.add2 = add2; a.a2 = a2;
  a.dx = dx; a.partial = c.w.ln_partial + c.w.ln_region * c.n_ln; a.M = c.d.M; a.D = c.d.D; a.K = K; a.dtype = c.d.dtype;
  a.variant = c.io->force_generic == 2 ? 1 : 0; a.x_lowp = c.d.rlow;
  uvc_ln_reduce_item& it = c.ln_items[c.n_ln++];
  it.partial = a.partial; it.dgamma = c.io->grads + pw; it.dbeta = c.io->grads + pb; it.dots = dots; it.nblocks = uvc_gemm_lnbwd_nblocks(c.d.M); it.reserved = 0;
  return uvc_gemm_nt_lnbwd(&a, c.st);
}
int attn(const Ctx& c, const BlockBufs& b, bool bwd, int layer = -1) {
  uvc_attn_args a;
  memset(&a, 0, sizeof(a));
  if (layer >= 0 && c.io->head_keep && (bwd ? c.io->head_keep_bwd != 0 : !c.io->training)) a.head_keep = c.io->head_keep + (size_t)layer * c.d.H;
  a.qkv = b.qkv; a.o = b.o; a.lse = b.lse; a.dout = c.w.dH; a.dqkv = c.w.dqkv; a.delta = c.w.delta;
  a.B = c.d.B; a.N = c.d.N; a.H = c.d.H; a.head_dim = 64; a.dtype = c.d.dtype; a.scale = 0.125f;
  return bwd ? uvc_attention_bwd(&a, c.st) : uvc_attention_fwd(&a, c.st);
}

int attn_tok(const Ctx& c, const BlockBufs& b, bool bwd, int layer = -1) {
  uvc_attn_tok_args a;
  memset(&a, 0, sizeof(a));
  if (layer >= 0 && c.io->head_keep && (bwd ? c.io->head_keep_bwd != 0 : !c.io->training)) a.head_keep = c.io->head_keep + (size_t)layer * c.d.H;
  a.qkv = b.qkv; a.o = c.w.tail.oc; a.dout = c.w.tail.dOc; a.dqkv = c.w.dqkv;
  a.B = c.d.B; a.N = c.d.N; a.H = c.d.H; a.head_dim = 64; a.ntok = c.d.ntok; a.dtype = c.d.dtype; a.scale = 0.125f;
  return bwd ? uvc_attention_tok_bwd(&a, c.st) : uvc_attention_tok_fwd(&a, c.st);
}
bool gp_q8(const Ctx& c, int rows, int Fe) {
  if (c.io->gelu_grad_bf16 || c.io->force_generic == 1) return false;
  if (c.io->fused_train_mlp && uvc_mlp_fused_supported(c.d.D, Fe, c.d.dtype)) return false;
  return uvc_gemm_nt_q8_supported(rows, Fe, c.d.D, c.d.dtype) != 0;
}
int gather_tok(const Ctx& c, const void* full, void* compact, size_t esz) {
  return uvc_copy_row_groups(full, compact, c.d.B, (int64_t)c.d.ntok * c.d.D * esz, (int64_t)c.d.N * c.d.D * esz, (int64_t)c.d.ntok * c.d.D * esz, c.st);
}
int scatter_tok(const Ctx& c, const void* compact, void* full, size_t esz) {
  return uvc_copy_row_groups(compact, full, c.d.B, (int64_t)c.d.ntok * c.d.D * esz, (int64_t)c.d.ntok * c.d.D * esz, (int64_t)c.d.N * c.d.D * esz, c.st);
}
int tail_block(const Ctx& c) {
  if (c.io->full_tail || c.d.N > 256 || c.d.ntok > 2) return -1;
  int last = -1;
  for (int l = 0; l < c.d.L; ++l)
    if (c.io->gate_d || !c.io->run_block || c.io->run_block[l] != 0) last = l;
  return last;
}

int setup(Ctx& c, const uvc_vit_cfg* cfg, const uvc_vit_io* io, void* stream, bool bwd) {
  TRY(check_cfg(cfg));
  if (!io || !io->params || !io->workspace || io->batch <= 0) return uvc_set_error_msg(UVC_ERR_ARG, "uvc_vit: null io member");
  if (cfg->dtype == UVC_BF16 && !io->shadow) return uvc_set_error_msg(UVC_ERR_ARG, "uvc_vit: bf16 mode needs the shadow buffer");
  if (!io->shadow) return uvc_set_error_msg(UVC_ERR_ARG, "uvc_vit: shadow buffer (W^T copies) missing");
  c.cfg = cfg; c.io = io; c.st = stream; c.d = dims_of(*cfg, io->batch);
  c.side = bwd ? io->side_stream : nullptr;
  c.n_pend = 0; c.tn_inline = false;
  if (c.side) TRY(ensure_events());
  TRY(uvc_vit_layout(cfg, &c.off, &c.soff));
  const int mode = (bwd || io->training) ? (io->shared_bwd_streams ? 2 : 1) : 0;
  if (mode == 2 && c.side) return uvc_set_error_msg(UVC_ERR_ARG, "uvc_vit: shared_bwd_streams (workspace mode 2) cannot be combined with a side stream");
  const int64_t need = carve(c.d, mode, (char*)io->workspace, c.w);
  if (io->workspace_bytes < need) return uvc_set_error_msg(UVC_ERR_ARG, "uvc_vit: workspace too small");
  if (io->patches_in) c.w.patches = const_cast<void*>(io->patches_in);
  return UVC_OK;
}

}

extern "C" int uvc_vit_layout(const uvc_vit_cfg* cfg, uvc_vit_offsets* off, uvc_vit_shadow_offsets* soff) {
  TRY(check_cfg(cfg));
  const Dims d = dims_of(*cfg, 1);
  if (off) {
    memset(off, 0xff, sizeof(*off));
    Slots put{0, 4};
    layout_embed(d, off, put);
    for (int l = 0; l < d.L; ++l) {
      int64_t* b = off->blk[l];
      put(b[0], d.D); put(b[1], d.D); put(b[2], (int64_t)3 * d.D * d.D); put(b[3], 3 * d.D); put(b[4], (int64_t)d.D * d.D); put(b[5], d.D);
      put(b[6], d.D); put(b[7], d.D); put(b[8], (int64_t)d.F * d.D); put(b[9], d.F); put(b[10], (int64_t)d.D * d.F); put(b[11], d.D);
    }
    layout_heads(d, off, put);
    put(off->gate, 2 * d.L);
    put(off->gumbel_w, d.D); put(off->gumbel_b, 1);
    put(off->patch_gating, d.np);
    for (int l = 0; l < d.L; ++l) { put(off->skip[l][0], 2); put(off->skip[l][1], 2); }
    off->n_total = put.o;
  }
  if (soff) {
    memset(soff, 0xff, sizeof(*soff));
    Slots put{0, 8};
    put(soff->patch_w, (int64_t)d.D * d.K0);
    const int64_t sz[4] = {(int64_t)3 * d.D * d.D, (int64_t)d.D * d.D, (int64_t)d.F * d.D, (int64_t)d.D * d.F};
    for (int l = 0; l < d.L; ++l)
      for (int j = 0; j < 4; ++j) { put(soff->blk_w[l][j], sz[j]); put(soff->blk_wt[l][j], sz[j]); }
// ... 192 lines not shown

extern "C" int uvc_vit_backward(const uvc_vit_cfg* cfg, const uvc_vit_io* io, void* stream) {
  Ctx c;
  memset(&c.w, 0, sizeof(c.w));
  TRY(setup(c, cfg, io, stream, true));
  if (!io->grads || !io->d_logits || (cfg->ntok == 2 && !io->d_logits_dist)) return uvc_set_error_msg(UVC_ERR_ARG, "uvc_vit_backward: null io member");
  const Dims& d = c.d;
  const float* P = io->params;
  float* G = io->grads;
  const uvc_vit_offsets& o = c.off;
  const uvc_vit_shadow_offsets& so = c.soff;
  Work& w = c.w;
  hipStream_t hs = (hipStream_t)stream;
  const int rh = d.B * d.ntok;
  const int gf = d.dtype == UVC_F32 ? 1 : 0;
  const int sb = io->stage_begin, se = (io->stage_begin == 0 && io->stage_end == 0) ? d.L + 3 : io->stage_end;
  if (sb < 0 || se > d.L + 3 || sb >= se) return uvc_set_error_msg(UVC_ERR_ARG, "uvc_vit_backward: bad stage range");
  const int tl = tail_block(c);
  const TailBufs& t = w.tail;
  auto runs = [&](int l) { return io->gate_d || !io->run_block || io->run_block[l]; };
  auto g_in = [&](int l) { int k = l + 1; while (k < d.L && !runs(k)) ++k; return w.gAs[k]; };
  if (io->shared_bwd_streams) {
    int cnt = 0;
    w.gAs[d.L] = w.gA_pp[0];
    for (int l = d.L - 1; l >= 0; --l) { if (runs(l)) ++cnt; w.gAs[l] = w.gA_pp[cnt & 1]; }
  }
  w.gA = w.gAs[d.L];
  int last_l = -1;
  for (int l = 0; l < d.L; ++l) { const int stage = d.L - l; if (stage >= sb && stage < se && runs(l)) { last_l = l; break; } }
  if (sb == 0) {
  TRY(nt(c, io->d_logits, 1, sh(c, so.head_wt), w.dhc, 0, d.B, d.D, d.NC, UVC_EPI_NONE, nullptr, nullptr, nullptr, nullptr, nullptr, nullptr, nullptr, 0,
         d.ntok * d.D));
  TRY(tn(c, io->d_logits, 1, w.hc, G + o.head_w, G + o.head_b, d.B, d.NC, d.D, nullptr, 0, d.ntok * d.D));
  if (d.ntok == 2) {
    TRY(nt(c, io->d_logits_dist, 1, sh(c, so.headd_wt), (char*)w.dhc + (size_t)d.D * d.tsz, 0, d.B, d.D, d.NC, UVC_EPI_NONE, nullptr, nullptr, nullptr,
           nullptr, nullptr, nullptr, nullptr, 0, d.ntok * d.D));
    TRY(tn(c, io->d_logits_dist, 1, (const char*)w.hc + (size_t)d.D * d.tsz, G + o.headd_w, G + o.headd_b, d.B, d.NC, d.D, nullptr, 0, d.ntok * d.D));
  }
  hipError_t he = hipMemsetAsync(w.gA, 0, (size_t)d.M * d.D * d.tsz, hs);
  if (he != hipSuccess) return uvc_set_error(he, __FILE__, __LINE__);
  if (tl >= 0) {
    TRY(ln_bwd(c, w.dhc, t.xoutc, o.norm_w, o.norm_b, w.meanf, w.rstdf, t.gAc, nullptr, nullptr, nullptr, nullptr, w.dotsraw + 2 * d.L, rh, 1, d.D));
    TRY(scatter_tok(c, t.gAc, w.gA, d.tsz));
  } else
  TRY(ln_bwd(c, w.dhc, w.xL, o.norm_w, o.norm_b, w.meanf, w.rstdf, w.gA, nullptr, nullptr, nullptr, nullptr, w.dotsraw + 2 * d.L, rh, d.ntok,
             (int64_t)d.N * d.D));
  }
  for (int l = d.L - 1; l >= 0; --l) {
    const int stage = d.L - l;
    if (stage < sb || stage >= se) continue;
    if (!io->gate_d && io->run_block && !io->run_block[l]) continue;
    const BlockBufs& b = w.blk[l];
    const int64_t* q = o.blk[l];
    const float* g0 = io->gate_d ? io->gate_d + 2 * l : nullptr;
    const float* g1 = io->gate_d ? io->gate_d + 2 * l + 1 : nullptr;
    const bool tail = l == tl;
    const int rows = tail ? d.B * d.ntok : d.M;
    void* const gA_in = g_in(l);
    w.gA = w.gAs[l]; w.gB = w.gBs[l]; w.dA = w.dAs[l]; w.dqkv = w.dqkvs[l];
    void* gA = tail ? t.gAc : gA_in; void* gB = tail ? t.gBc : w.gB; void* dA = tail ? t.dAc : w.dA; void* dH = tail ? t.dHc : w.dH;
    const void* fa = tail ? t.ac : b.a; const void* fu = tail ? t.uc : b.u; const void* fh2 = tail ? t.h2c : b.h2;
    const void* fx1 = tail ? t.x1c : b.x1; const float* fm2 = tail ? t.mean2c : b.mean2; const float* fr2 = tail ? t.rstd2c : b.rstd2;
    const uvc_mlp_compact* mc = (io->mlp_compact && io->mlp_compact[l].width > 0 && io->mlp_compact[l].width < d.F) ? &io->mlp_compact[l] : nullptr;
    const bool fuse2 = !mc && !tail && lnb_fused_ok(c, d.F);
    c.tn_inline = c.side && l == last_l && !mc;
    if (!mc) {
      TRY(nt(c, gA, gf, sh(c, so.blk_wt[l][3]), dA, 0, rows, d.F, d.D, gp_q8(c, rows, d.F) ? UVC_EPI_MUL_AUX_Q8 : UVC_EPI_MUL_AUX, nullptr, nullptr, nullptr, fa, nullptr,
             nullptr, g1));
      TRY(tn(c, gA, gf, fu, G + q[10], G + q[11], rows, d.D, d.F, g1));
      if (!fuse2) TRY(nt(c, dA, 0, sh(c, so.blk_wt[l][2]), dH, 0, rows, d.D, d.F, UVC_EPI_NONE));
      TRY(tn(c, dA, 0, fh2, G + q[8], G + q[9], rows, d.F, d.D));
    } else {
      const int Fe = mc->width;
      if (io->accumulate != 0.f) return uvc_set_error_msg(UVC_ERR_UNSUPPORTED, "uvc_vit_backward: gradient accumulation with MLP compaction");
      TRY(nt(c, gA, gf, mc->w2t, dA, 0, rows, Fe, d.D, gp_q8(c, rows, Fe) ? UVC_EPI_MUL_AUX_Q8 : UVC_EPI_MUL_AUX, nullptr, nullptr, nullptr, fa, nullptr, nullptr, g1));
      TRY(tn(c, gA, gf, fu, mc->dw2, G + q[11], rows, d.D, Fe, g1, 0, 0, true));
      TRY(nt(c, dA, 0, mc->w1t, dH, 0, rows, d.D, Fe, UVC_EPI_NONE));
      TRY(tn(c, dA, 0, fh2, mc->dw1, mc->db1, rows, Fe, d.D, nullptr, 0, 0, true));
      TRY(flush_tn(c));
      TRY(uvc_mlp_scatter_grads(mc->dw1, mc->dw2, mc->db1, mc->inv, P + q[9], G + q[11], d.D, d.F, Fe, G + q[8], G + q[10], G + q[9], 0.f, d.dtype,
                                c.side ? c.side : c.st));
    }
    c.tn_inline = false;
    if (fuse2)
      TRY(dgrad_ln_bwd(c, w.dA, sh(c, so.blk_wt[l][2]), d.F, b.x1, q[6], q[7], b.mean2, b.rstd2, w.gB, gA_in, g1, nullptr, nullptr, nullptr));
    else
    TRY(ln_bwd(c, dH, fx1, q[6], q[7], fm2, fr2, gB, gA, g1, nullptr, nullptr, nullptr, rows, 1, d.D));
    TRY(nt(c, gB, gf, sh(c, so.blk_wt[l][1]), tail ? t.dOc : w.dH, 0, rows, d.D, d.D, UVC_EPI_NONE));
    TRY(tn(c, gB, gf, tail ? t.oc : b.o, G + q[4], G + q[5], rows, d.D, d.D));
    if (tail) {
      TRY(attn_tok(c, b, true, l));
      const hipError_t he = hipMemsetAsync(w.gB, 0, (size_t)d.M * d.D * d.tsz, hs);
      if (he != hipSuccess) return uvc_set_error(he, __FILE__, __LINE__);
      TRY(scatter_tok(c, t.gBc, w.gB, d.tsz));
    } else
    TRY(attn(c, b, true, l));
    const bool fuse1 = lnb_fused_ok(c, 3 * d.D);
    if (!fuse1) TRY(nt(c, w.dqkv, 0, sh(c, so.blk_wt[l][0]), w.dH, 0, d.M, d.D, 3 * d.D, UVC_EPI_NONE));
    TRY(tn(c, w.dqkv, 0, b.h1, G + q[2], d.qkv_bias ? G + q[3] : nullptr, d.M, 3 * d.D, d.D));
    if (fuse1)
      TRY(dgrad_ln_bwd(c, w.dqkv, sh(c, so.blk_wt[l][0]), 3 * d.D, b.x, q[0], q[1], b.mean1, b.rstd1, w.gA, w.gB, nullptr, io->gate_d ? gA_in : nullptr, g0,
                       w.dotsraw + 2 * l));
    else
    TRY(ln_bwd(c, w.dH, b.x, q[0], q[1], b.mean1, b.rstd1, w.gA, w.gB, nullptr, io->gate_d ? gA_in : nullptr, g0, w.dotsraw + 2 * l, d.M, 1, d.D));
    TRY(flush_tn(c));
  }
  w.gA = g_in(-1);
  if (sb <= d.L + 1 && se > d.L + 1) {
    TRY(flush_ln(c));
    if (io->gate_d && io->gate_mode != 0)
      TRY(uvc_gate_grad(P + o.gate, io->gate_d, w.dotsraw, G + o.gate, d.L, io->gate_mode, io->gate_eps, io->accumulate, stream));
    TRY(uvc_assemble_tokens_bwd(w.gA, w.pe, io->patch_mask, w.dpe, G + o.pos_embed, G + o.cls_token, d.ntok == 2 ? G + o.dist_token : nullptr,
                                io->d_patch_mask, d.B, d.np, d.D, d.ntok, d.dtype, 0, d.dtype == UVC_BF16, io->accumulate, stream));
  }
  TRY(flush_ln(c));
  if (se < d.L + 3) return join_side(c);
  TRY(tn(c, w.dpe, 0, w.patches, G + o.patch_w, G + o.patch_b, d.B * d.np, d.D, d.K0));
  return join_side(c);
}
```

### uvc_amd/model_distilled.py

```python
from __future__ import annotations

import ctypes as C
import os
from functools import partial
from typing import Optional

import numpy as np
import torch
import torch.nn as nn

from . import _lib as L
from . import ops

__all__ = ["DistilledVisionTransformer", "PatchEmbed", "Attention", "Mlp", "Block"]


class uvc_vit_cfg(C.Structure):
    _fields_ = [(n, C.c_int32) for n in ("img_size", "patch_size", "in_chans", "num_classes", "embed_dim", "depth",
                                         "num_heads", "hidden", "ntok", "dtype")] + [("ln_eps", C.c_float), ("no_qkv_bias", C.c_int32),
                                                                                       ("resid_f32", C.c_int32), ("reserved", C.c_int32)]


MAXD = 32


class uvc_vit_offsets(C.Structure):
    _fields_ = [(n, C.c_int64) for n in ("cls_token", "dist_token", "pos_embed", "patch_w", "patch_b")] + \
               [("blk", (C.c_int64 * 12) * MAXD)] + \
               [(n, C.c_int64) for n in ("norm_w", "norm_b", "head_w", "head_b", "headd_w", "headd_b", "n_main", "gate",
                                         "gumbel_w", "gumbel_b", "patch_gating")] + \
               [("skip", (C.c_int64 * 2) * MAXD), ("n_total", C.c_int64)]


class uvc_vit_shadow_offsets(C.Structure):
    _fields_ = [("patch_w", C.c_int64), ("blk_w", (C.c_int64 * 4) * MAXD), ("blk_wt", (C.c_int64 * 4) * MAXD)] + \
               [(n, C.c_int64) for n in ("head_w", "head_wt", "headd_w", "headd_wt", "n_total")]


class uvc_vit_io(C.Structure):
    _fields_ = [("params", C.c_void_p), ("shadow", C.c_void_p), ("grads", C.c_void_p), ("workspace", C.c_void_p),
                ("workspace_bytes", C.c_int64), ("x", C.c_void_p), ("logits", C.c_void_p), ("logits_dist", C.c_void_p),
                ("d_logits", C.c_void_p), ("d_logits_dist", C.c_void_p), ("gate_d", C.c_void_p),
                ("run_block", C.POINTER(C.c_int32)), ("patch_mask", C.c_void_p), ("d_patch_mask", C.c_void_p),
                ("batch", C.c_int32), ("training", C.c_int32), ("gate_mode", C.c_int32), ("gate_eps", C.c_float),
                ("accumulate", C.c_float), ("stage_begin", C.c_int32), ("stage_end", C.c_int32), ("side_stream", C.c_void_p),
                ("mlp_compact", C.c_void_p), ("head_keep", C.c_void_p), ("full_tail", C.c_int32), ("fused_train_mlp", C.c_int32), ("patches_in", C.c_void_p),
                ("fuse_next_ln", C.c_int32), ("force_generic", C.c_int32), ("head_keep_bwd", C.c_int32), ("shared_bwd_streams", C.c_int32),
                ("gelu_grad_bf16", C.c_int32)]


class uvc_mlp_compact(C.Structure):
    _fields_ = [("width", C.c_int32), ("reserved", C.c_int32)] + \
               [(n, C.c_void_p) for n in ("w1", "w1t", "w2", "w2t", "b1", "dw1", "dw2", "db1", "inv")]


_FULL_TAIL_DEFAULT = os.environ.get("UVC_FULL_TAIL", "0") not in ("", "0")
_GELU_GRAD_BF16_DEFAULT = os.environ.get("UVC_GELU_GRAD_BF16", "0") not in ("", "0")
_FUSE_NEXT_LN_DEFAULT = os.environ.get("UVC_FUSE_NEXT_LN", "1") not in ("", "0")
_RESID_F32_DEFAULT = os.environ.get("UVC_RESID_F32", "0") not in ("", "0")
_FUSED_TRAIN_MLP_DEFAULT = os.environ.get("UVC_FUSED_TRAIN_MLP", "0") not in ("", "0")


_SHARE_PATCHES = os.environ.get("UVC_SHARE_PATCHES", "1") not in ("", "0")
_PATCH_SHARE = dict(x=None, key=None, buf=None, ev=None, owner=None)


def _shared_patches(model, x, x_key=None):
    cfg = model._cfg
    x_key = x if x_key is None else x_key
    key = (x_key._version, tuple(x.shape), cfg.patch_size, model.precision)
    c = _PATCH_SHARE
    cur = torch.cuda.current_stream()
    if _SHARE_PATCHES and c["x"] is x_key and c["key"] == key and c["owner"] != id(model):
        buf, ev = c["buf"], c["ev"]
        c.update(x=None, key=None, buf=None, ev=None, owner=None)
        cur.wait_event(ev)
        buf.record_stream(cur)
        return buf
    B = x.shape[0]
    rows = B * (cfg.img_size // cfg.patch_size) ** 2
    buf = torch.empty(rows, cfg.in_chans * cfg.patch_size * cfg.patch_size, device=x.device,
                      dtype=torch.float32 if model.precision == "fp32" else torch.bfloat16)
    ops.patchify(x, buf, cfg.patch_size, ops.UVC_F32 if model.precision == "fp32" else ops.UVC_BF16)
    if _SHARE_PATCHES:
        ev = torch.cuda.Event()
        ev.record(cur)
        c.update(x=x_key, key=key, buf=buf, ev=ev, owner=id(model))
    return buf


def drop_shared_patches():
    _PATCH_SHARE.update(x=None, key=None, buf=None, ev=None, owner=None)


def _bind():
    lib = L.lib()
    if getattr(lib, "_vit_bound", False):
        return lib
    lib.uvc_vit_layout.argtypes = [C.POINTER(uvc_vit_cfg), C.POINTER(uvc_vit_offsets), C.POINTER(uvc_vit_shadow_offsets)]
    lib.uvc_vit_layout.restype = C.c_int
    lib.uvc_vit_workspace_bytes.argtypes = [C.POINTER(uvc_vit_cfg), C.c_int32, C.c_int32]
    lib.uvc_vit_workspace_bytes.restype = C.c_int64
    lib.uvc_vit_update_shadows.argtypes = [C.POINTER(uvc_vit_cfg), C.c_void_p, C.c_void_p, C.c_void_p]
    lib.uvc_vit_update_shadows.restype = C.c_int
    for n in ("uvc_vit_forward", "uvc_vit_backward"):
        f = getattr(lib, n)
        f.argtypes = [C.POINTER(uvc_vit_cfg), C.POINTER(uvc_vit_io), C.c_void_p]
        f.restype = C.c_int
    lib._vit_bound = True
    return lib


VIT_SYMBOLS = ["uvc_vit_layout", "uvc_vit_workspace_bytes", "uvc_vit_update_shadows", "uvc_vit_forward", "uvc_vit_backward"]


class PatchEmbed(nn.Module):

    def __init__(self, img_size=224, patch_size=16, in_chans=3, embed_dim=768):
        super().__init__()
        self.img_size = (img_size, img_size)
        self.patch_size = (patch_size, patch_size)
        self.grid_size = (img_size // patch_size, img_size // patch_size)
        self.num_patches = self.grid_size[0] * self.grid_size[1]
        self.proj = nn.Conv2d(in_chans, embed_dim, kernel_size=patch_size, stride=patch_size)


class Attention(nn.Module):
    def __init__(self, dim, num_heads=8, qkv_bias=False):
        super().__init__()
        self.num_heads = num_heads
        self.scale = (dim // num_heads) ** -0.5
        self.qkv = nn.Linear(dim, dim * 3, bias=qkv_bias)
        self.proj = nn.Linear(dim, dim)


class Mlp(nn.Module):
    def __init__(self, in_features, hidden_features=None):
        super().__init__()
        self.fc1 = nn.Linear(in_features, hidden_features)
        self.act = nn.GELU()
# ... 273 lines not shown
        self._shadow_fresh = False
        return widths

    def set_head_skipping(self, keep=None):
        self._head_keep_derived = keep is None
        if keep is False:
            self._head_keep = None
            return None
        cfg = self._cfg
        if keep is None:
            rows = []
            for blk in self.blocks:
                m = getattr(blk.attn.proj, "mask", None)
                rows.append(torch.ones(cfg.num_heads, dtype=torch.bool) if m is None else
                            (m != 0).any(dim=0).reshape(cfg.num_heads, -1).any(dim=1).cpu())
            keep = torch.stack(rows)
        keep = keep.to(torch.int32).contiguous()
        self._head_keep = None if bool(keep.all()) else keep.to(self._flat.device)
        return keep

    def _gather_compact(self):
        dt = ops.UVC_F32 if self.precision == "fp32" else ops.UVC_BF16
        cfg = self._cfg
        for blk, b in zip(self.blocks, self._mlp_bufs):
            if b is None:
                continue
            ops.mlp_gather_shadows(blk.mlp.fc1.weight.data, blk.mlp.fc1.bias.data, blk.mlp.fc2.weight.data, b["idx"], b["w1"], b["w1t"],
                                   b["w2"], b["w2t"], b["b1"], cfg.embed_dim, cfg.hidden, b["width"], dt)

    def apply_masks(self):
        self._check_flat()
        ops.apply_masks(self._flat, self._mask_flat())
        self.mark_weights_changed()

    def load_state_dict(self, *a, **k):
        r = super().load_state_dict(*a, **k)
        self.mark_weights_changed()
        self._run_block_host = None
        if getattr(self, "_head_keep_derived", False):
            self.set_head_skipping()
        if getattr(self, "_mlp_compact_derived", None) is not None:
            self.set_mlp_compaction(multiple=self._mlp_compact_derived)
        return r

    def _ws_mode(self, training):
        if not training:
            return 0
        return 1 if self.two_stream_backward else 2

    def _workspace(self, B, training):
        mode = self._ws_mode(training)
        key = (B, bool(training), mode)
        if key not in self._ws:
            nbytes = _bind().uvc_vit_workspace_bytes(C.byref(self._cfg), B, mode)
            if nbytes < 0:
                raise L.UvcHipError(f"uvc_vit_workspace_bytes: {L.lib().uvc_last_error().decode()}")
            self._ws = {k: v for k, v in self._ws.items() if k[1] != bool(training)}
            self._ws[key] = torch.empty(nbytes, device=self._flat.device, dtype=torch.uint8)
        return self._ws[key]

    def _gate_mode(self):
        if not self.enable_block_gating or self.enable_warmup:
            return 0
        return 1 if self.use_gumbel == 1 else 2

    def _io(self, B, training):
        io = uvc_vit_io()
        ws = self._workspace(B, training)
        io.params, io.shadow, io.grads = L.ptr(self._flat), L.ptr(self._shadow), L.ptr(self._flat_grad)
        io.workspace, io.workspace_bytes = L.ptr(ws), ws.numel()
        io.batch, io.training = B, int(training)
        io.shared_bwd_streams = int(self._ws_mode(training) == 2)
        io.gate_mode, io.gate_eps = self._gate_mode(), float(self.eps)
        io.accumulate = 1.0 if self.grad_accumulate else 0.0
        io.mlp_compact = C.addressof(self._mlp_compact) if self._mlp_compact is not None else None
        skip_bwd = bool(training and getattr(self, "skip_pruned_head_grads", False))
        io.head_keep = L.ptr(self._head_keep) if (self._head_keep is not None and (not training or skip_bwd)) else None
        io.head_keep_bwd = int(skip_bwd and self._head_keep is not None)
        io.full_tail = int(getattr(self, "full_tail", _FULL_TAIL_DEFAULT))
        io.fused_train_mlp = int(getattr(self, "fused_train_mlp", _FUSED_TRAIN_MLP_DEFAULT))
        io.fuse_next_ln = int(getattr(self, "fuse_next_ln", _FUSE_NEXT_LN_DEFAULT))
        io.force_generic = int(getattr(self, "force_generic", 0))
        io.gelu_grad_bf16 = int(getattr(self, "gelu_grad_bf16", _GELU_GRAD_BF16_DEFAULT))
        return io

    def _ws_view(self, B, training, which):
        lib = _bind()
        if not hasattr(lib, "_wsoff_bound"):
            lib.uvc_vit_ws_offsets.argtypes = [C.POINTER(uvc_vit_cfg), C.c_int32, C.c_int32, C.POINTER(C.c_int64), C.POINTER(C.c_int64)]
            lib.uvc_vit_ws_offsets.restype = C.c_int
            lib._wsoff_bound = True
        pe_off, dpe_off = C.c_int64(), C.c_int64()
        L.check(lib.uvc_vit_ws_offsets(C.byref(self._cfg), B, self._ws_mode(training), C.byref(pe_off), C.byref(dpe_off)), "uvc_vit_ws_offsets")
        ws = self._workspace(B, training)
        cfg = self._cfg
        rows = B * (cfg.img_size // cfg.patch_size) ** 2
        if which == "pe":
            return ws[pe_off.value:pe_off.value + rows * cfg.embed_dim * 4].view(torch.float32).view(rows, cfg.embed_dim)
        tdt = torch.float32 if self.precision == "fp32" else torch.bfloat16
        nb = rows * cfg.embed_dim * (4 if self.precision == "fp32" else 2)
        return ws[dpe_off.value:dpe_off.value + nb].view(tdt).view(rows, cfg.embed_dim)

    def _run_forward(self, x, tau, ratio, training):
        L.require_cuda(x)
        x_key = x
        if x.dtype != torch.float32 or not x.is_contiguous():
            x = x.contiguous().float()
        B = x.shape[0]
        cfg = self._cfg
        if tuple(x.shape[1:]) != (cfg.in_chans, cfg.img_size, cfg.img_size):
            raise AssertionError(f"Input image size ({x.shape[2]}*{x.shape[3]}) doesn't match model ({cfg.img_size}*{cfg.img_size}).")
        self._check_flat()
        lib = _bind()
        stream = L.cur_stream()
        if not (self.frozen_weights and self._shadow_fresh):
            L.check(lib.uvc_vit_update_shadows(C.byref(cfg), L.ptr(self._flat), L.ptr(self._shadow), stream), "uvc_vit_update_shadows")
            if self._mlp_compact is not None:
                self._gather_compact()
            self._shadow_fresh = True
        io = self._io(B, training)
        dev = self._flat.device
        logits = torch.empty(B, cfg.num_classes, device=dev)
        logits_dist = torch.empty(B, cfg.num_classes, device=dev) if self.num_tokens == 2 else None
        gate_d = None
        run_block = None
        if self.enable_block_gating:
            gate_d = torch.empty(cfg.depth, 2, device=dev)
            if self.enable_warmup:
                mode = 0
            elif self.use_gumbel == 1:
                mode = 3 if self.gumbel_hard else 1
            else:
                mode = 2
        else:
            run_block = self._hard_run_blocks()
        io.x, io.logits, io.logits_dist = L.ptr(x), L.ptr(logits), L.ptr(logits_dist)
        io.run_block = run_block if run_block is not None else None
        P = (cfg.img_size // cfg.patch_size) ** 2
        mode1 = self.enable_patch_gating == 1
        mode2 = tau > 0
        if mode1 and mode2:
            raise NotImplementedError("patch gating modes 1 and 2 together (never produced by the reference driver)")
        patch = None
        front = self._front_end_forward(x, B, training)
        patches = None
        if front:
            io.stage_begin, io.stage_end = 1, 2
        else:
            patches = _shared_patches(self, x, x_key)
            io.patches_in = L.ptr(patches)
        if mode1 or mode2:
            if not front:
                io.stage_begin, io.stage_end = 0, 1
                L.check(lib.uvc_vit_forward(C.byref(cfg), C.byref(io), stream), "uvc_vit_forward")
            mask = torch.empty(B, P, device=dev)
            if mode1:
                ops.patch_gate_sigmoid(self.patch_gating.data, mask, B, P, self.patch_hard)
                patch = dict(mode=1, mask=mask)
            else:
                pe = self._ws_view(B, training, "pe")
                scores, ys, ps = (torch.empty(B, P, device=dev) for _ in range(3))
                ops.patch_scores(pe, self.gumbel.weight.data, self.gumbel.bias.data, scores, B * P, cfg.embed_dim)
                ops.patch_topk_mask(scores, self.exp_source((B, P)), mask, ys, ps, B, P, int(ratio * P), float(tau))
                patch = dict(mode=2, mask=mask, ysoft=ys, psoft=ps, tau=float(tau))
            io.patch_mask = L.ptr(mask)
            io.stage_begin, io.stage_end = 1, 2
# ... 133 lines not shown
```

### uvc_amd/ops.py

```python
from __future__ import annotations

import ctypes as C
from typing import Optional

import torch

from . import _lib as L
from ._lib import (EPI_BIAS, EPI_BIAS_GELU, EPI_BIAS_GELU_GRAD, EPI_BIAS_GELU_GRAD_Q8, EPI_BIAS_GELU_OUT, EPI_BIAS_RESID, EPI_BIAS_RESID_GATE, EPI_DGELU,
                   EPI_MUL_AUX, EPI_MUL_AUX_Q8, EPI_NONE, Q8_LO, Q8_STEP, UVC_BF16, UVC_F32)

__all__ = ["EPI_NONE", "EPI_BIAS", "EPI_BIAS_GELU", "EPI_BIAS_RESID", "EPI_BIAS_RESID_GATE", "EPI_DGELU", "UVC_F32",
           "UVC_BF16"]


def tdtype(dtype: int) -> torch.dtype:
    return torch.float32 if dtype == UVC_F32 else torch.bfloat16


def _chk(*ts):
    for t in ts:
        if t is None:
            continue
        L.require_cuda(t)
        if not t.is_contiguous():
# ... 108 lines not shown
    a.dout, a.dqkv = L.ptr(dout), L.ptr(dqkv)
    a.B, a.N, a.H, a.head_dim, a.ntok, a.dtype, a.scale = B, N, H, 64, ntok, dtype, 0.125
    return a


def attention_tok_fwd(qkv, o, B, N, H, ntok, dtype, head_keep=None):
    a = _attn_tok_args(qkv, o, B, N, H, ntok, dtype)
    if head_keep is not None:
        _chk(head_keep)
        a.head_keep = L.ptr(head_keep)
    L.check(L.lib().uvc_attention_tok_fwd(C.byref(a), L.cur_stream()), "uvc_attention_tok_fwd")


def attention_tok_bwd(qkv, o, dout, dqkv, B, N, H, ntok, dtype):
    a = _attn_tok_args(qkv, o, B, N, H, ntok, dtype, dout, dqkv)
    L.check(L.lib().uvc_attention_tok_bwd(C.byref(a), L.cur_stream()), "uvc_attention_tok_bwd")


def copy_row_groups(src, dst, groups, group_bytes, src_group_stride, dst_group_stride):
    _chk(src)
    _chk(dst)
    L.check(L.lib().uvc_copy_row_groups(L.ptr(src), L.ptr(dst), groups, group_bytes, src_group_stride, dst_group_stride, L.cur_stream()),
            "uvc_copy_row_groups")


def _ln_args(x, gamma, beta, rows, D, dtype, rows_per_group=1, group_stride=None, eps=1e-6):
    a = L.uvc_ln_args()
    a.x, a.gamma, a.beta = L.ptr(x), L.ptr(gamma), L.ptr(beta)
    a.rows, a.D, a.rows_per_group, a.dtype = rows, D, rows_per_group, dtype
    a.group_stride = group_stride if group_stride is not None else D * rows_per_group
    a.eps = eps
    a.x_lowp = int(not _is_f32(x))
    return a


def layernorm_fwd(x, gamma, beta, y, mean, rstd, rows, D, dtype, rows_per_group=1, group_stride=None, eps=1e-6):
    _chk(x, gamma, beta, y, mean, rstd)
    a = _ln_args(x, gamma, beta, rows, D, dtype, rows_per_group, group_stride, eps)
    a.y, a.mean, a.rstd, a.y_is_f32 = L.ptr(y), L.ptr(mean), L.ptr(rstd), _is_f32(y)
    L.check(L.lib().uvc_layernorm_fwd(C.byref(a), L.cur_stream()), "uvc_layernorm_fwd")


def layernorm_bwd_blocks(rows) -> int:
    return int(L.lib().uvc_layernorm_bwd_blocks(rows))


def layernorm_bwd(dy, x, gamma, mean, rstd, dx, partial, dgamma, dbeta, rows, D, dtype, *, add1=None, a1=None, add2=None,
                  a2=None, dots=None, beta_acc=0.0, rows_per_group=1, group_stride=None, eps=1e-6):
    _chk(dy, x, gamma, mean, rstd, dx, partial, dgamma, dbeta, add1, a1, add2, a2, dots)
    a = _ln_args(x, gamma, None, rows, D, dtype, rows_per_group, group_stride, eps)
    a.mean, a.rstd, a.dy, a.dx = L.ptr(mean), L.ptr(rstd), L.ptr(dy), L.ptr(dx)
    a.add1, a.a1, a.add2, a.a2 = L.ptr(add1), L.ptr(a1), L.ptr(add2), L.ptr(a2)
    a.partial, a.dgamma, a.dbeta, a.dots = L.ptr(partial), L.ptr(dgamma), L.ptr(dbeta), L.ptr(dots)
    a.beta_acc, a.dy_is_f32 = beta_acc, _is_f32(dy)
    a.g_lowp = int(not _is_f32(dx))
    for t in (add1, add2):
        if t is not None and t.dtype != dx.dtype:
            raise L.UvcHipError("layernorm_bwd: add1/add2 must have dx's element type")
    L.check(L.lib().uvc_layernorm_bwd(C.byref(a), L.cur_stream()), "uvc_layernorm_bwd")


def gemm_nt_q8_supported(M, hidden, embed_dim, dtype) -> bool:
    return bool(L.lib().uvc_gemm_nt_q8_supported(M, hidden, embed_dim, dtype))


def gemm_lnbwd_supported(M, D, K, dtype) -> bool:
    return bool(L.lib().uvc_gemm_lnbwd_supported(M, D, K, dtype))


def gemm_nt_lnbwd(A, Wt, x, mean, rstd, gamma, dx, partial, dgamma, dbeta, *, add1=None, a1=None, add2=None, a2=None, dots=None, beta_acc=0.0,
                  variant=0):
    _chk(A, Wt, x, mean, rstd, gamma, dx, partial, dgamma, dbeta, add1, a1, add2, a2, dots)
    a = L.uvc_gemm_lnbwd_args()
    a.A, a.W, a.x, a.mean, a.rstd, a.gamma = (L.ptr(t) for t in (A, Wt, x, mean, rstd, gamma))
    a.add1, a.a1, a.add2, a.a2, a.dx, a.partial = (L.ptr(t) for t in (add1, a1, add2, a2, dx, partial))
    a.M, a.D, a.K, a.dtype, a.variant, a.x_lowp = A.shape[0], x.shape[1], A.shape[1], UVC_BF16, int(variant), int(not _is_f32(x))
    L.check(L.lib().uvc_gemm_nt_lnbwd(C.byref(a), L.cur_stream()), "uvc_gemm_nt_lnbwd")
    item = (L.uvc_ln_reduce_item * 1)()
    item[0].partial, item[0].dgamma, item[0].dbeta, item[0].dots = L.ptr(partial), L.ptr(dgamma), L.ptr(dbeta), L.ptr(dots)
    item[0].nblocks = int(L.lib().uvc_gemm_lnbwd_nblocks(a.M))
    L.check(L.lib().uvc_layernorm_bwd_reduce_batch(item, 1, a.D, beta_acc, L.cur_stream()), "uvc_layernorm_bwd_reduce_batch")


def mlp_fused_fwd(x, gamma, beta, w1, b1, w2, b2, out, eps=1e-6, *, x_prev=None, gate=None, h=None, mean=None, rstd=None, gp=None, u=None,
                  next_gamma=None, next_beta=None, next_h=None, next_mean=None, next_rstd=None):
    _chk(x, gamma, beta, w1, b1, w2, b2, out, x_prev, gate, h, mean, rstd, gp, u, next_gamma, next_beta, next_h, next_mean, next_rstd)
    a = L.uvc_mlp_args()
    a.next_gamma, a.next_beta, a.next_h, a.next_mean, a.next_rstd = (L.ptr(t) for t in (next_gamma, next_beta, next_h, next_mean, next_rstd))
    a.x, a.gamma, a.beta, a.w1, a.b1, a.w2, a.b2, a.out = (L.ptr(t) for t in (x, gamma, beta, w1, b1, w2, b2, out))
    a.x_prev, a.gate, a.h, a.mean, a.rstd, a.gp, a.u = (L.ptr(t) for t in (x_prev, gate, h, mean, rstd, gp, u))
    a.M, a.D, a.F, a.eps = x.shape[0], x.shape[1], w1.shape[0], eps
    a.rows_lowp = int(not _is_f32(x))
    for t in (out, x_prev):
        if t is not None and t.dtype != x.dtype:
            raise L.UvcHipError("mlp_fused_fwd: x, out and x_prev must share one element type")
    L.check(L.lib().uvc_mlp_fused_fwd(C.byref(a), L.cur_stream()), "uvc_mlp_fused_fwd")


def distill_loss(o, o_kd, y_soft, teacher, loss, d_o, d_okd, row_scratch, alpha, tau, kind=1):
    _chk(o, o_kd, y_soft, teacher, loss, d_o, d_okd, row_scratch)
    a = L.uvc_loss_args()
    a.o, a.o_kd, a.y_soft, a.teacher = L.ptr(o), L.ptr(o_kd), L.ptr(y_soft), L.ptr(teacher)
    a.loss, a.d_o, a.d_okd, a.row_scratch = L.ptr(loss), L.ptr(d_o), L.ptr(d_okd), L.ptr(row_scratch)
    a.alpha, a.tau, a.B, a.C, a.kind = alpha, tau, o.shape[0], o.shape[1], kind
    L.check(L.lib().uvc_distill_loss(C.byref(a), L.cur_stream()), "uvc_distill_loss")


def grad_sqnorm(g, partial, sq, accumulate=False, n=None):
    _chk(g, partial, sq)
    if sq.numel() < 2:
        raise L.UvcHipError("grad_sqnorm: sq must hold 2 floats (sum of squares, norm)")
    L.check(L.lib().uvc_grad_sqnorm(L.ptr(g), n if n is not None else g.numel(), L.ptr(partial), L.ptr(sq),
                                    int(accumulate), L.cur_stream()), "uvc_grad_sqnorm")


def adamw_step(p, g, m, v, sq, *, lr, step, beta1=0.9, beta2=0.999, eps=1e-8, weight_decay=0.05, max_norm=1.0,
               p_shadow=None, gnorm_out=None, n=None, flags=None):
    _chk(p, g, m, v, sq, p_shadow, gnorm_out, flags)
    a = L.uvc_adamw_args()
    a.p, a.g, a.m, a.v, a.p_shadow, a.sq, a.gnorm_out = (L.ptr(t) for t in (p, g, m, v, p_shadow, sq, gnorm_out))
    a.n = n if n is not None else p.numel()
    a.lr, a.beta1, a.beta2, a.eps, a.weight_decay, a.max_norm, a.step = lr, beta1, beta2, eps, weight_decay, max_norm, step
    a.flags = L.ptr(flags)
    L.check(L.lib().uvc_adamw_step(C.byref(a), L.cur_stream()), "uvc_adamw_step")


def scale_by_clip(g, sq, max_norm):
    _chk(g, sq)
    L.check(L.lib().uvc_scale_by_clip(L.ptr(g), g.numel(), L.ptr(sq), max_norm, L.cur_stream()), "uvc_scale_by_clip")


def patchify(x, out, P, dtype):
    _chk(x, out)
    B, Cc, S, _ = x.shape
    L.check(L.lib().uvc_patchify(L.ptr(x), L.ptr(out), B, Cc, S, P, dtype, L.cur_stream()), "uvc_patchify")


def assemble_tokens(pe, cls, dist, pos, row_mask, tok, B, P, D, ntok):
    _chk(pe, cls, dist, pos, row_mask, tok)
    L.check(L.lib().uvc_assemble_tokens(L.ptr(pe), L.ptr(cls), L.ptr(dist), L.ptr(pos), L.ptr(row_mask), L.ptr(tok), B, P,
                                        D, ntok, int(not _is_f32(tok)), L.cur_stream()), "uvc_assemble_tokens")


def assemble_tokens_bwd(dtok, pe, row_mask, dpe, dpos, dcls, ddist, dmask, B, P, D, ntok, dtype, beta_acc=0.0):
    _chk(dtok, pe, row_mask, dpe, dpos, dcls, ddist, dmask)
    L.check(L.lib().uvc_assemble_tokens_bwd(L.ptr(dtok), L.ptr(pe), L.ptr(row_mask), L.ptr(dpe), L.ptr(dpos), L.ptr(dcls),
                                            L.ptr(ddist), L.ptr(dmask), B, P, D, ntok, dtype, _is_f32(dpe), int(not _is_f32(dtok)), beta_acc,
                                            L.cur_stream()), "uvc_assemble_tokens_bwd")


def colsum_blocks(M) -> int:
    return int(L.lib().uvc_colsum_blocks(M))


def colsum(X, partial, out, dtype, *, M=None, N=None, ldx=None, alpha=1.0, alpha_ptr=None, beta=0.0, row_weight=None):
    _chk(X, partial, out, alpha_ptr, row_weight)
    M = M if M is not None else X.shape[0]
    N = N if N is not None else X.shape[1]
    L.check(L.lib().uvc_colsum(L.ptr(X), M, N, ldx if ldx is not None else N, dtype, _is_f32(X), L.ptr(partial), L.ptr(out),
                               alpha, L.ptr(alpha_ptr), beta, L.ptr(row_weight), L.cur_stream()), "uvc_colsum")


def patch_gate_sigmoid(pg, mask, B, P, hard):
    _chk(pg, mask)
    L.check(L.lib().uvc_patch_gate_sigmoid(L.ptr(pg), L.ptr(mask), B, P, int(bool(hard)), L.cur_stream()), "uvc_patch_gate_sigmoid")

# ... 224 lines not shown
```

Measured before the change: 47770 images/sec.

## Fuse attention-proj dgrad GEMM into the dfc1 + LayerNorm2 backward kernel

Adds a PROJ variant of the warp-specialised dfc1+LayerNorm-backward kernel. It keeps the proj weight (192x192) in registers, stages each finished dx tile in LDS, and multiplies it by the proj weight one tile behind, interleaved with the main GEMM's k-loop. This removes the separate proj dgrad GEMM launch and its re-read of gB from global memory in each block's backward pass. The cost is more register pressure and extra LDS in an already tightly scheduled kernel, plus lane-index recomputation tricks. It can be disabled with UVC_SPLIT_DPROJ.

```diff
diff --git a/include/uvc_kernels.h b/include/uvc_kernels.h
--- a/include/uvc_kernels.h
+++ b/include/uvc_kernels.h
@@ -147,6 +147,13 @@
 int uvc_gemm_lnbwd_supported(int32_t M, int32_t D, int32_t K, int32_t dtype);
 int uvc_gemm_lnbwd_nblocks(int32_t M);
 int uvc_gemm_nt_lnbwd(const uvc_gemm_lnbwd_args* args, void* stream);
+typedef struct uvc_gemm_lnbwd_proj_args {
+  uvc_gemm_lnbwd_args ln;
+  const void* W2;
+  void* out2;
+} uvc_gemm_lnbwd_proj_args;
+int uvc_gemm_lnbwd_proj_supported(int32_t M, int32_t D, int32_t K, int32_t dtype);
+int uvc_gemm_nt_lnbwd_proj(const uvc_gemm_lnbwd_proj_args* args, void* stream);
 
 typedef struct uvc_mlp_args {
   const void* x; const float* gamma; const float* beta;
diff --git a/include/uvc_vit.h b/include/uvc_vit.h
--- a/include/uvc_vit.h
+++ b/include/uvc_vit.h
@@ -82,6 +82,7 @@
   int32_t head_keep_bwd;
   int32_t shared_bwd_streams;
   int32_t gelu_grad_bf16;
+  int32_t split_dproj;
 } uvc_vit_io;
 
 int uvc_vit_forward(const uvc_vit_cfg* cfg, const uvc_vit_io* io, void* stream);
diff --git a/uvc_amd/_lib.py b/uvc_amd/_lib.py
--- a/uvc_amd/_lib.py
+++ b/uvc_amd/_lib.py
@@ -83,6 +83,10 @@
 class uvc_gemm_lnbwd_args(C.Structure):
     _fields_ = [(n, C.c_void_p) for n in ("A", "W", "x", "mean", "rstd", "gamma", "add1", "a1", "add2", "a2", "dx", "partial")] + \
                [(n, C.c_int32) for n in ("M", "D", "K", "dtype", "variant", "x_lowp")]
+
+
+class uvc_gemm_lnbwd_proj_args(C.Structure):
+    _fields_ = [("ln", uvc_gemm_lnbwd_args), ("W2", C.c_void_p), ("out2", C.c_void_p)]
 
 
 class uvc_mlp_args(C.Structure):
@@ -192,6 +196,8 @@
     "uvc_gemm_lnbwd_supported": [I32, I32, I32, I32],
     "uvc_gemm_lnbwd_nblocks": [I32],
     "uvc_gemm_nt_lnbwd": [C.POINTER(uvc_gemm_lnbwd_args), VP],
+    "uvc_gemm_lnbwd_proj_supported": [I32, I32, I32, I32],
+    "uvc_gemm_nt_lnbwd_proj": [C.POINTER(uvc_gemm_lnbwd_proj_args), VP],
     "uvc_distill_loss": [C.POINTER(uvc_loss_args), VP],
     "uvc_grad_sqnorm": [VP, I64, VP, VP, I32, VP],
     "uvc_adamw_step": [C.POINTER(uvc_adamw_args), VP],
diff --git a/uvc_amd/csrc/gemm.hip b/uvc_amd/csrc/gemm.hip
--- a/uvc_amd/csrc/gemm.hip
+++ b/uvc_amd/csrc/gemm.hip
@@ -1096,6 +1096,7 @@
   const void* A; const void* W; const void* x; const float* mean; const float* rstd; const float* gamma;
   const void* add1; const float* a1; const void* add2; const float* a2; void* dx; float* partial;
   int M, K, want_dots;
+  const void* W2; void* out2;
 };
 
 template <int KT, bool XLOW>
@@ -1260,7 +1261,7 @@
 template <int N> __device__ __forceinline__ void wait_vm() { asm volatile("s_waitcnt vmcnt(%0)" ::"n"(N) : "memory"); }
 #define TIE4(a, b, c, d) asm volatile("" : "+v"(a), "+v"(b), "+v"(c), "+v"(d))
 
-template <int KT, bool HAS2, bool XLOW>
+template <int KT, bool HAS2, bool XLOW, bool PROJ = false>
 __global__ __launch_bounds__(768) void k_gemm_wsn_lnbwd_dma(LnbArgs g) {
   typedef bf16_t T;
   typedef Mma<T> MM;
@@ -1274,7 +1275,9 @@
   constexpr int STAGE = NI * 1024;
   static_assert((16 * SA) % 64 == 32, "spare half block behind the A image");
   constexpr int MR_OFF = (NA - 1) * 1024 + 512;
-  static_assert(NI <= 5 * NWV && 3 * STAGE + 2 * 16 * NWV * 8 + D * 4 <= 160 * 1024, "ring does not fit");
+  constexpr int EXB = PS * 16, EX_OFF = 3 * STAGE + 2 * 16 * NWV * 8 + D * 4;
+  static_assert(NI <= 5 * NWV && EX_OFF + (PROJ ? 2 * 16 * EXB : 0) <= 160 * 1024, "ring does not fit");
+  static_assert(!PROJ || (KT == 24 && !HAS2 && XLOW), "the proj dgrad rides on dfc1 + LayerNorm2' only");
   extern __shared__ __attribute__((aligned(16))) char smem[];
   float* sRed = reinterpret_cast<float*>(smem + 3 * STAGE);
   const int tid = threadIdx.x, lane = tid & 63, gq = lane >> 4, li = lane & 15;
@@ -1323,14 +1326,36 @@
   const long long mr_delta = reinterpret_cast<const char*>(g.rstd) - reinterpret_cast<const char*>(g.mean);
   const unsigned mr_lo = (unsigned)(lane & 3) * 16u;
   const bool mr_lane = lane >= 32 && lane < 40, mr_r = lane >= 36;
+  static_assert(16 * K * 2 <= 65536, "lane offsets of a tile fit 16 bits");
+  const unsigned loffp[3] = {PROJ ? loff[0] | loff[1] << 16 : 0u, PROJ ? loff[2] | loff[3] << 16 : 0u, PROJ ? loff[4] : 0u};
   auto issue_q = [&](int tile, int st, int q) {
     const int t = tile < ntiles ? tile : ntiles - 1;
     if (q < 5) {
-      const char* src = rb[q] + ((unsigned long long)(unsigned)t * (unsigned long long)rstride[q] + (unsigned long long)loff[q]);
+      const char* src;
+      if constexpr (PROJ) {
+        const unsigned long long sb64 = (unsigned long long)rb[q] + (unsigned long long)(unsigned)t * (unsigned long long)rstride[q];
+        const unsigned lo = __builtin_amdgcn_readfirstlane((unsigned)sb64), hi = __builtin_amdgcn_readfirstlane((unsigned)(sb64 >> 32));
+        unsigned vo = loffp[q >> 1];
+        asm volatile("" : "+v"(vo));
+        vo = (q & 1) ? vo >> 16 : vo & 0xffffu;
+        asm volatile("" : "+v"(vo));
+        src = reinterpret_cast<const char*>(((unsigned long long)hi << 32) | lo) + (unsigned long long)vo;
+      } else
+      src = rb[q] + ((unsigned long long)(unsigned)t * (unsigned long long)rstride[q] + (unsigned long long)loff[q]);
       char* dst = smem + st * STAGE + rdst[q];
       __builtin_amdgcn_global_load_lds((const void __attribute__((address_space(1)))*)src, (void __attribute__((address_space(3)))*)dst, 16, 0, 0);
     } else if (mr_lane) {
-      const char* src = reinterpret_cast<const char*>(g.mean) + ((unsigned long long)(unsigned)t * 64ull + mr_lo) + (mr_r ? mr_delta : 0ll);
+      const char* src;
+      if constexpr (PROJ) {
+        const unsigned long long sb64 = (unsigned long long)(mr_delta >= 0 ? g.mean : g.rstd) + (unsigned long long)(unsigned)t * 64ull;
+        const unsigned lo = __builtin_amdgcn_readfirstlane((unsigned)sb64), hi = __builtin_amdgcn_readfirstlane((unsigned)(sb64 >> 32));
+        int l = lane;
+        asm volatile("" : "+v"(l));
+        unsigned vo = (unsigned)(l & 3) * 16u + (((l >= 36) == (mr_delta >= 0)) ? (unsigned)(mr_delta >= 0 ? mr_delta : -mr_delta) : 0u);
+        asm volatile("" : "+v"(vo));
+        src = reinterpret_cast<const char*>(((unsigned long long)hi << 32) | lo) + (unsigned long long)vo;
+      } else
+      src = reinterpret_cast<const char*>(g.mean) + ((unsigned long long)(unsigned)t * 64ull + mr_lo) + (mr_r ? mr_delta : 0ll);
       char* dst = smem + st * STAGE + (NA - 1) * 1024;
       __builtin_amdgcn_global_load_lds((const void __attribute__((address_space(1)))*)src, (void __attribute__((address_space(3)))*)dst, 16, 0, 0);
     }
@@ -1343,6 +1368,37 @@
   const unsigned fragoff = (unsigned)(li * ROWB + gq * 16);
   const unsigned xoff = (unsigned)(I_X * 1024 + li * XB + n * XSZ), poff = (unsigned)(I_1 * 1024 + li * PB + n * 2), moff = (unsigned)(MR_OFF + li * 4);
   const unsigned redr = lds_addr(sRed) + (unsigned)(li * NWV * 8);
+  struct LaneIdx { int li, gq, n; };
+  auto lane_here = [&]() -> LaneIdx {
+    if constexpr (!PROJ) return LaneIdx{li, gq, n};
+    int l = lane;
+    asm volatile("" : "+v"(l));
+    return LaneIdx{l & 15, l >> 4, w * 16 + (l >> 4) * 4};
+  };
+  u32x4 wp[PROJ ? D / 32 : 1];
+  if constexpr (PROJ) {
+    const LaneIdx LW = lane_here();
+#pragma unroll
+    for (int ks = 0; ks < D / 32; ++ks)
+      wp[ks] = *reinterpret_cast<const u32x4*>(reinterpret_cast<const T*>(g.W2) + (size_t)(w * 16 + LW.li) * D + (ks * 4 + LW.gq) * 8);
+    asm volatile("" : "+v"(wp[0]), "+v"(wp[1]), "+v"(wp[2]), "+v"(wp[3]), "+v"(wp[4]), "+v"(wp[5]));
+  }
+  auto proj_tile = [&](int ptile, int p) {
+    const LaneIdx LD = lane_here();
+    const unsigned er = s0 + (unsigned)(EX_OFF + p * 16 * EXB) + (unsigned)(LD.li * EXB + LD.gq * 16);
+    u32x4 ea[2];
+    f32x4 acc = {0.f, 0.f, 0.f, 0.f};
+#define PROJ2(KS) ea[0] = ds_read128<(KS) * 64>(er); ea[1] = ds_read128<(KS) * 64 + 64>(er); wait_lgkm<0>(); \
+    asm volatile("" : "+v"(ea[0]), "+v"(ea[1])); \
+    acc = MM::mma(__builtin_bit_cast(typename MM::Frag, wp[KS]), __builtin_bit_cast(typename MM::Frag, ea[0]), acc); \
+    acc = MM::mma(__builtin_bit_cast(typename MM::Frag, wp[(KS) + 1]), __builtin_bit_cast(typename MM::Frag, ea[1]), acc);
+    PROJ2(0) PROJ2(2) PROJ2(4)
+#undef PROJ2
+#pragma unroll
+    for (int e = 0; e < 4; ++e) acc[e] = epi_scale_bias(acc[e], 1.0f, 0.0f);
+    u32x2 q; q[0] = pack_bf16x2(acc[0], acc[1]); q[1] = pack_bf16x2(acc[2], acc[3]);
+    *reinterpret_cast<u32x2*>(reinterpret_cast<T*>(g.out2) + ((size_t)(ptile * 16 + LD.li) * D + LD.n)) = q;
+  };
 
   int tile = blockIdx.x;
   issue(tile, 0);
@@ -1356,17 +1412,26 @@
     f32x4 c0 = {0.f, 0.f, 0.f, 0.f};
     constexpr bool DB = KT <= 18;
     u32x4 fa[2], fb[2];
-    const unsigned fr = sb + fragoff;
+    const LaneIdx LA = lane_here();
+    const unsigned fr = sb + (PROJ ? (unsigned)(LA.li * ROWB + LA.gq * 16) : fragoff);
+    const unsigned er = s0 + (unsigned)(EX_OFF + par * 16 * EXB) + (unsigned)(LA.li * EXB + LA.gq * 16);
+    f32x4 acc = {0.f, 0.f, 0.f, 0.f};
 #define RD2(dst, ks0) dst[0] = ds_read128<(ks0) * 64>(fr); dst[1] = ds_read128<(ks0) * 64 + 64>(fr);
 #define GROUP(gk, cur, nxt) if ((gk) < KT / 2) { \
       if (DB) { if ((gk) + 1 < KT / 2) { RD2(nxt, ((gk) + 1) * 2) wait_lgkm<2>(); } else wait_lgkm<0>(); \
                 asm volatile("" : "+v"(cur[0]), "+v"(cur[1])); \
                 c0 = MM::mma(bf[(gk) * 2], __builtin_bit_cast(typename MM::Frag, cur[0]), c0); \
                 c0 = MM::mma(bf[(gk) * 2 + 1], __builtin_bit_cast(typename MM::Frag, cur[1]), c0); } \
+      else if (PROJ && (gk) % 4 == 1) {  \
+             wait_lgkm<0>(); \
+             asm volatile("" : "+v"(fa[0]), "+v"(fa[1])); \
+             acc = MM::mma(__builtin_bit_cast(typename MM::Frag, wp[PROJ ? (gk) / 4 * 2 : 0]), __builtin_bit_cast(typename MM::Frag, fa[0]), acc); \
+             acc = MM::mma(__builtin_bit_cast(typename MM::Frag, wp[PROJ ? (gk) / 4 * 2 + 1 : 0]), __builtin_bit_cast(typename MM::Frag, fa[1]), acc); } \
       else if (((gk) & 1) == 0) { RD2(fa, (gk) * 2) RD2(fb, (gk) * 2 + 2) wait_lgkm<0>();  \
              asm volatile("" : "+v"(fa[0]), "+v"(fa[1]), "+v"(fb[0]), "+v"(fb[1])); \
              c0 = MM::mma(bf[(gk) * 2], __builtin_bit_cast(typename MM::Frag, fa[0]), c0); \
              c0 = MM::mma(bf[(gk) * 2 + 1], __builtin_bit_cast(typename MM::Frag, fa[1]), c0); \
+             if (PROJ && (gk) % 4 == 0) { fa[0] = ds_read128<(gk) / 4 * 128>(er); fa[1] = ds_read128<(gk) / 4 * 128 + 64>(er); } \
              c0 = MM::mma(bf[(gk) * 2 + 2], __builtin_bit_cast(typename MM::Frag, fb[0]), c0); \
              c0 = MM::mma(bf[(gk) * 2 + 3], __builtin_bit_cast(typename MM::Frag, fb[1]), c0); } }
     static_assert(KT % 2 == 0 && KT <= 24, "pairs of k-steps");
@@ -1376,16 +1441,29 @@
     GROUP(8, fa, fb) issue_q(nt_, ns_, 4); issue_q(nt_, ns_, 5); GROUP(9, fb, fa) GROUP(10, fa, fb) GROUP(11, fb, fa)
 #undef GROUP
 #undef RD2
+    if constexpr (PROJ) {
+      if (tile - 2 * (int)gridDim.x >= (int)blockIdx.x) {
+        const LaneIdx LS = lane_here();
+#pragma unroll
+        for (int e = 0; e < 4; ++e) acc[e] = epi_scale_bias(acc[e], 1.0f, 0.0f);
+        u32x2 q; q[0] = pack_bf16x2(acc[0], acc[1]); q[1] = pack_bf16x2(acc[2], acc[3]);
+        *reinterpret_cast<u32x2*>(reinterpret_cast<T*>(g.out2) + ((size_t)((tile - 2 * (int)gridDim.x) * 16 + LS.li) * D + LS.n)) = q;
+      }
+    }
+    const LaneIdx LB = lane_here();
+    const unsigned xoff_ = PROJ ? (unsigned)(I_X * 1024 + LB.li * XB + LB.n * XSZ) : xoff, poff_ = PROJ ? (unsigned)(I_1 * 1024 + LB.li * PB + LB.n * 2) : poff;
+    const unsigned moff_ = PROJ ? (unsigned)(MR_OFF + LB.li * 4) : moff, gaddr_ = PROJ ? lds_addr(sGam) + (unsigned)LB.n * 4u : gaddr;
+    const unsigned redr_ = PROJ ? lds_addr(sRed) + (unsigned)(LB.li * NWV * 8) : redr;
     typename Resid<typename std::conditional<XLOW, bf16_t, float>::type>::Raw4 xr;
-    if constexpr (XLOW) asm volatile("ds_read_b64 %0, %1" : "=v"(xr) : "v"(sb + xoff));
-    else xr = ds_read128<0>(sb + xoff);
+    if constexpr (XLOW) asm volatile("ds_read_b64 %0, %1" : "=v"(xr) : "v"(sb + xoff_));
+    else xr = ds_read128<0>(sb + xoff_);
     u32x2 r1 = {0u, 0u}, r2 = {0u, 0u};
-    if (has1) asm volatile("ds_read_b64 %0, %1" : "=v"(r1) : "v"(sb + poff));
-    if (has2) asm volatile("ds_read_b64 %0, %1 offset:%2" : "=v"(r2) : "v"(sb + poff), "n"((I_2 - I_1) * 1024));
+    if (has1) asm volatile("ds_read_b64 %0, %1" : "=v"(r1) : "v"(sb + poff_));
+    if (has2) asm volatile("ds_read_b64 %0, %1 offset:%2" : "=v"(r2) : "v"(sb + poff_), "n"((I_2 - I_1) * 1024));
     float mean, rstd;
-    asm volatile("ds_read_b32 %0, %1" : "=v"(mean) : "v"(sb + moff));
-    asm volatile("ds_read_b32 %0, %1 offset:64" : "=v"(rstd) : "v"(sb + moff));
-    u32x4 gr = ds_read128<0>(gaddr);
+    asm volatile("ds_read_b32 %0, %1" : "=v"(mean) : "v"(sb + moff_));
+    asm volatile("ds_read_b32 %0, %1 offset:64" : "=v"(rstd) : "v"(sb + moff_));
+    u32x4 gr = ds_read128<0>(gaddr_);
     wait_lgkm<0>();
     asm volatile("" : "+v"(xr), "+v"(r1), "+v"(r2), "+v"(mean), "+v"(rstd), "+v"(gr));
     const f32x4 xv = Resid<typename std::conditional<XLOW, bf16_t, float>::type>::f4(xr);
@@ -1403,7 +1481,7 @@
       }
       p1 = sum_rows4(p1);
       p2 = sum_rows4(p2);
-      if (gq == 0) ds_write64_a(redr + (unsigned)(par * 16 * NWV * 8 + w * 8), f32x2{p1, p2});
+      if (LB.gq == 0) ds_write64_a(redr_ + (unsigned)(par * 16 * NWV * 8 + w * 8), f32x2{p1, p2});
 #pragma unroll
       for (int e = 0; e < 4; ++e) c0[e] *= gam[e];
     }
@@ -1411,8 +1489,9 @@
     wait_lgkm<0>();
     __builtin_amdgcn_s_barrier();
     float c1 = 0.f, c2 = 0.f;
+    const LaneIdx LC = lane_here();
     {
-      const unsigned rr = redr + (unsigned)(par * 16 * NWV * 8);
+      const unsigned rr = (PROJ ? lds_addr(sRed) + (unsigned)(LC.li * NWV * 8) : redr) + (unsigned)(par * 16 * NWV * 8);
       u32x4 t0 = ds_read128<0>(rr), t1 = ds_read128<16>(rr), t2 = ds_read128<32>(rr);
       wait_lgkm<0>();
       asm volatile("" : "+v"(t0), "+v"(t1), "+v"(t2));
@@ -1430,6 +1509,8 @@
     }
     c1 *= invD; c2 *= invD;
     {
+      if constexpr (PROJ) asm volatile("" : "+v"(xr));
+      const f32x4 xv = Resid<typename std::conditional<XLOW, bf16_t, float>::type>::f4(xr);
       const f32x4 v1 = {__uint_as_float(r1[0] << 16), __uint_as_float(r1[0] & 0xffff0000u), __uint_as_float(r1[1] << 16), __uint_as_float(r1[1] & 0xffff0000u)};
       const f32x4 v2 = {__uint_as_float(r2[0] << 16), __uint_as_float(r2[0] & 0xffff0000u), __uint_as_float(r2[1] << 16), __uint_as_float(r2[1] & 0xffff0000u)};
       float o[4];
@@ -1442,22 +1523,33 @@
         dotA += o[e] * xv[e];
       }
       u32x2 q; q[0] = pack_bf16x2(o[0], o[1]); q[1] = pack_bf16x2(o[2], o[3]);
-      *reinterpret_cast<u32x2*>(dx + ((size_t)(tile * 16 + li) * D + n)) = q;
+      *reinterpret_cast<u32x2*>(dx + ((size_t)(tile * 16 + LC.li) * D + LC.n)) = q;
+      if constexpr (PROJ) {
+        const unsigned ew = s0 + (unsigned)(EX_OFF + par * 16 * EXB) + (unsigned)(LC.li * EXB + LC.n * 2);
+        asm volatile("ds_write_b64 %0, %1" ::"v"(ew), "v"(q) : "memory");
+      }
     }
     st = st == 2 ? 0 : st + 1;
     par ^= 1;
   }
   wait_vm<0>();
+  if constexpr (PROJ) wait_lgkm<0>();
   __syncthreads();
+  if constexpr (PROJ) {
+    const int last = tile - (int)gridDim.x;
+    if (last - (int)gridDim.x >= (int)blockIdx.x) proj_tile(last - (int)gridDim.x, par);
+    proj_tile(last, par ^ 1);
+  }
 #pragma unroll
   for (int e = 0; e < 4; ++e) {
 #pragma unroll
     for (int o = 1; o < 16; o <<= 1) { dgam[e] += __shfl_xor(dgam[e], o, 64); dbet[e] += __shfl_xor(dbet[e], o, 64); }
   }
   float* P = g.partial + (size_t)blockIdx.x * (2 * D + 2);
-  if (li == 0) {
-    *reinterpret_cast<f32x2*>(P + n) = f32x2{dgam[0], dgam[1]}; *reinterpret_cast<f32x2*>(P + n + 2) = f32x2{dgam[2], dgam[3]};
-    *reinterpret_cast<f32x2*>(P + D + n) = f32x2{dbet[0], dbet[1]}; *reinterpret_cast<f32x2*>(P + D + n + 2) = f32x2{dbet[2], dbet[3]};
+  const LaneIdx LE = lane_here();
+  if (LE.li == 0) {
+    *reinterpret_cast<f32x2*>(P + LE.n) = f32x2{dgam[0], dgam[1]}; *reinterpret_cast<f32x2*>(P + LE.n + 2) = f32x2{dgam[2], dgam[3]};
+    *reinterpret_cast<f32x2*>(P + D + LE.n) = f32x2{dbet[0], dbet[1]}; *reinterpret_cast<f32x2*>(P + D + LE.n + 2) = f32x2{dbet[2], dbet[3]};
   }
   dotA = wave_sum(dotA); dotB = wave_sum(dotB);
   if (lane == 0) { sRed[2 * w] = dotA; sRed[2 * w + 1] = dotB; }
@@ -1720,7 +1812,7 @@
     return uvc_set_error_msg(UVC_ERR_ARG, "uvc_gemm_nt_lnbwd: misaligned buffer");
   LnbArgs a;
   a.A = p->A; a.W = p->W; a.x = p->x; a.mean = p->mean; a.rstd = p->rstd; a.gamma = p->gamma; a.add1 = p->add1; a.a1 = p->a1;
-  a.add2 = p->add2; a.a2 = p->a2; a.dx = p->dx; a.partial = p->partial; a.M = p->M; a.K = p->K; a.want_dots = 1;
+  a.add2 = p->add2; a.a2 = p->a2; a.dx = p->dx; a.partial = p->partial; a.M = p->M; a.K = p->K; a.want_dots = 1; a.W2 = nullptr; a.out2 = nullptr;
   const int grid = uvc_gemm_lnbwd_nblocks(p->M);
   hipStream_t st = (hipStream_t)stream;
   if (p->D == 384) return launch_row384_lnbwd(a, p->x_lowp, st);
@@ -1742,6 +1834,35 @@
 #undef LNB_LAUNCH_DMA
 #undef LNB_DMA_ONE
 #undef LNB_LAUNCH
+  UVC_CHECK_LAUNCH();
+  return UVC_OK;
+}
+
+extern "C" int uvc_gemm_lnbwd_proj_supported(int32_t M, int32_t D, int32_t K, int32_t dtype) {
+  return dtype == UVC_BF16 && D == 192 && K == 768 && M >= 4096 && M % 16 == 0;
+}
+
+extern "C" int uvc_gemm_nt_lnbwd_proj(const uvc_gemm_lnbwd_proj_args* q, void* stream) {
+  if (!q) return uvc_set_error_msg(UVC_ERR_ARG, "uvc_gemm_nt_lnbwd_proj: null pointer");
+  const uvc_gemm_lnbwd_args* p = &q->ln;
+  if (!p->A || !p->W || !p->x || !p->mean || !p->rstd || !p->gamma || !p->dx || !p->partial || !q->W2 || !q->out2)
+    return uvc_set_error_msg(UVC_ERR_ARG, "uvc_gemm_nt_lnbwd_proj: null pointer");
+  const int64_t mr = (int64_t)((uintptr_t)p->rstd - (uintptr_t)p->mean);
+  const bool al16 = (((uintptr_t)p->A | (uintptr_t)p->W | (uintptr_t)p->x | (uintptr_t)p->gamma | (uintptr_t)p->add1 | (uintptr_t)p->mean | (uintptr_t)p->rstd |
+                      (uintptr_t)p->dx | (uintptr_t)q->W2 | (uintptr_t)q->out2) & 15) == 0 && ((uintptr_t)p->partial & 7) == 0;
+  if (!uvc_gemm_lnbwd_proj_supported(p->M, p->D, p->K, p->dtype) || !p->x_lowp || p->add2 || p->variant != 0 || !al16 || mr >= (1ll << 31) || mr <= -(1ll << 31))
+    return uvc_set_error_msg(UVC_ERR_UNSUPPORTED, "uvc_gemm_nt_lnbwd_proj: bf16 rows, M >= 4096, M % 16 == 0, D = 192, K = 768, no add2, 16-byte aligned operands");
+  if (q->out2 == p->dx || q->out2 == p->A || q->out2 == p->x || q->out2 == p->add1)
+    return uvc_set_error_msg(UVC_ERR_ARG, "uvc_gemm_nt_lnbwd_proj: out2 aliases an operand");
+  LnbArgs a;
+  a.A = p->A; a.W = p->W; a.x = p->x; a.mean = p->mean; a.rstd = p->rstd; a.gamma = p->gamma; a.add1 = p->add1; a.a1 = p->a1;
+  a.add2 = nullptr; a.a2 = nullptr; a.dx = p->dx; a.partial = p->partial; a.M = p->M; a.K = p->K; a.want_dots = 1; a.W2 = q->W2; a.out2 = q->out2;
+  const int grid = uvc_gemm_lnbwd_nblocks(p->M);
+  hipStream_t st = (hipStream_t)stream;
+  constexpr int NI_ = (16 * (24 * 4 + 2) + 63) / 64 + 7 + 7 + 7;
+  const size_t sh = (size_t)3 * NI_ * 1024 + (2 * 16 * 12 * 2 + 192) * sizeof(float) + 2 * 16 * 416;
+  UVC_MAX_LDS(sh, k_gemm_wsn_lnbwd_dma<24, false, true, true>);
+  k_gemm_wsn_lnbwd_dma<24, false, true, true><<<grid, 768, sh, st>>>(a);
   UVC_CHECK_LAUNCH();
   return UVC_OK;
 }
diff --git a/uvc_amd/csrc/vit_engine.hip b/uvc_amd/csrc/vit_engine.hip
--- a/uvc_amd/csrc/vit_engine.hip
+++ b/uvc_amd/csrc/vit_engine.hip
@@ -212,17 +212,23 @@
   return uvc_layernorm_bwd(&a, c.st);
 }
 bool lnb_fused_ok(const Ctx& c, int K) { return c.io->force_generic != 1 && uvc_gemm_lnbwd_supported(c.d.M, c.d.D, K, c.d.dtype) != 0; }
+bool proj_fused_ok(const Ctx& c, int K) {
+  return lnb_fused_ok(c, K) && c.io->force_generic == 0 && !c.io->split_dproj && c.d.rlow && uvc_gemm_lnbwd_proj_supported(c.d.M, c.d.D, K, c.d.dtype) != 0;
+}
 int dgrad_ln_bwd(Ctx& c, const void* A, const void* Wt, int K, const void* x, int64_t pw, int64_t pb, const float* mean, const float* rstd, void* dx,
-                 const void* add1, const float* a1, const void* add2, const float* a2, float* dots) {
+                 const void* add1, const float* a1, const void* add2, const float* a2, float* dots, const void* W2t = nullptr, void* out2 = nullptr) {
   if (c.n_ln >= 2 * c.d.L + 1) { if (int e = flush_ln(c)) return e; }
-  uvc_gemm_lnbwd_args a;
-  memset(&a, 0, sizeof(a));
+  uvc_gemm_lnbwd_proj_args ap;
+  memset(&ap, 0, sizeof(ap));
+  uvc_gemm_lnbwd_args& a = ap.ln;
   a.A = A; a.W = Wt; a.x = x; a.mean = mean; a.rstd = rstd; a.gamma = c.io->params + pw; a.add1 = add1; a.a1 = a1; a.add2 = add2; a.a2 = a2;
   a.dx = dx; a.partial = c.w.ln_partial + c.w.ln_region * c.n_ln; a.M = c.d.M; a.D = c.d.D; a.K = K; a.dtype = c.d.dtype;
   a.variant = c.io->force_generic == 2 ? 1 : 0; a.x_lowp = c.d.rlow;
   uvc_ln_reduce_item& it = c.ln_items[c.n_ln++];
   it.partial = a.partial; it.dgamma = c.io->grads + pw; it.dbeta = c.io->grads + pb; it.dots = dots; it.nblocks = uvc_gemm_lnbwd_nblocks(c.d.M); it.reserved = 0;
-  return uvc_gemm_nt_lnbwd(&a, c.st);
+  if (!W2t) return uvc_gemm_nt_lnbwd(&a, c.st);
+  ap.W2 = W2t; ap.out2 = out2;
+  return uvc_gemm_nt_lnbwd_proj(&ap, c.st);
 }
 int attn(const Ctx& c, const BlockBufs& b, bool bwd, int layer = -1) {
   uvc_attn_args a;
@@ -581,11 +587,15 @@
                                 c.side ? c.side : c.st));
     }
     c.tn_inline = false;
+    const bool fuse_dproj = fuse2 && proj_fused_ok(c, d.F) &&
+                            (((uintptr_t)w.dA | (uintptr_t)b.x1 | (uintptr_t)b.mean2 | (uintptr_t)b.rstd2 | (uintptr_t)w.gB | (uintptr_t)gA_in | (uintptr_t)w.dH |
+                              (uintptr_t)sh(c, so.blk_wt[l][1]) | (uintptr_t)sh(c, so.blk_wt[l][2]) | (uintptr_t)(c.io->params + q[6])) & 15) == 0;
     if (fuse2)
-      TRY(dgrad_ln_bwd(c, w.dA, sh(c, so.blk_wt[l][2]), d.F, b.x1, q[6], q[7], b.mean2, b.rstd2, w.gB, gA_in, g1, nullptr, nullptr, nullptr));
+      TRY(dgrad_ln_bwd(c, w.dA, sh(c, so.blk_wt[l][2]), d.F, b.x1, q[6], q[7], b.mean2, b.rstd2, w.gB, gA_in, g1, nullptr, nullptr, nullptr,
+                       fuse_dproj ? sh(c, so.blk_wt[l][1]) : nullptr, fuse_dproj ? w.dH : nullptr));
     else
     TRY(ln_bwd(c, dH, fx1, q[6], q[7], fm2, fr2, gB, gA, g1, nullptr, nullptr, nullptr, rows, 1, d.D));
-    TRY(nt(c, gB, gf, sh(c, so.blk_wt[l][1]), tail ? t.dOc : w.dH, 0, rows, d.D, d.D, UVC_EPI_NONE));
+    if (!fuse_dproj) TRY(nt(c, gB, gf, sh(c, so.blk_wt[l][1]), tail ? t.dOc : w.dH, 0, rows, d.D, d.D, UVC_EPI_NONE));
     TRY(tn(c, gB, gf, tail ? t.oc : b.o, G + q[4], G + q[5], rows, d.D, d.D));
     if (tail) {
       TRY(attn_tok(c, b, true, l));
diff --git a/uvc_amd/model_distilled.py b/uvc_amd/model_distilled.py
--- a/uvc_amd/model_distilled.py
+++ b/uvc_amd/model_distilled.py
@@ -46,7 +46,7 @@
                 ("accumulate", C.c_float), ("stage_begin", C.c_int32), ("stage_end", C.c_int32), ("side_stream", C.c_void_p),
                 ("mlp_compact", C.c_void_p), ("head_keep", C.c_void_p), ("full_tail", C.c_int32), ("fused_train_mlp", C.c_int32), ("patches_in", C.c_void_p),
                 ("fuse_next_ln", C.c_int32), ("force_generic", C.c_int32), ("head_keep_bwd", C.c_int32), ("shared_bwd_streams", C.c_int32),
-                ("gelu_grad_bf16", C.c_int32)]
+                ("gelu_grad_bf16", C.c_int32), ("split_dproj", C.c_int32)]
 
 
 class uvc_mlp_compact(C.Structure):
@@ -56,6 +56,7 @@
 
 _FULL_TAIL_DEFAULT = os.environ.get("UVC_FULL_TAIL", "0") not in ("", "0")
 _GELU_GRAD_BF16_DEFAULT = os.environ.get("UVC_GELU_GRAD_BF16", "0") not in ("", "0")
+_SPLIT_DPROJ_DEFAULT = os.environ.get("UVC_SPLIT_DPROJ", "0") not in ("", "0")
 _FUSE_NEXT_LN_DEFAULT = os.environ.get("UVC_FUSE_NEXT_LN", "1") not in ("", "0")
 _RESID_F32_DEFAULT = os.environ.get("UVC_RESID_F32", "0") not in ("", "0")
 _FUSED_TRAIN_MLP_DEFAULT = os.environ.get("UVC_FUSED_TRAIN_MLP", "0") not in ("", "0")
@@ -495,6 +496,7 @@
         io.fuse_next_ln = int(getattr(self, "fuse_next_ln", _FUSE_NEXT_LN_DEFAULT))
         io.force_generic = int(getattr(self, "force_generic", 0))
         io.gelu_grad_bf16 = int(getattr(self, "gelu_grad_bf16", _GELU_GRAD_BF16_DEFAULT))
+        io.split_dproj = int(getattr(self, "split_dproj", _SPLIT_DPROJ_DEFAULT))
         return io
 
     def _ws_view(self, B, training, which):
diff --git a/uvc_amd/ops.py b/uvc_amd/ops.py
--- a/uvc_amd/ops.py
+++ b/uvc_amd/ops.py
@@ -214,6 +214,23 @@
     L.check(L.lib().uvc_layernorm_bwd_reduce_batch(item, 1, a.D, beta_acc, L.cur_stream()), "uvc_layernorm_bwd_reduce_batch")
 
 
+def gemm_lnbwd_proj_supported(M, D, K, dtype) -> bool:
+    return bool(L.lib().uvc_gemm_lnbwd_proj_supported(M, D, K, dtype))
+
+
+def gemm_nt_lnbwd_proj(A, Wt, x, mean, rstd, gamma, dx, partial, W2t, out2, *, add1=None, a1=None, check=True):
+    _chk(A, Wt, x, mean, rstd, gamma, dx, partial, W2t, out2, add1, a1)
+    a = L.uvc_gemm_lnbwd_proj_args()
+    a.ln.A, a.ln.W, a.ln.x, a.ln.mean, a.ln.rstd, a.ln.gamma = (L.ptr(t) for t in (A, Wt, x, mean, rstd, gamma))
+    a.ln.add1, a.ln.a1, a.ln.dx, a.ln.partial = (L.ptr(t) for t in (add1, a1, dx, partial))
+    a.ln.M, a.ln.D, a.ln.K, a.ln.dtype, a.ln.variant, a.ln.x_lowp = A.shape[0], x.shape[1], A.shape[1], UVC_BF16, 0, int(not _is_f32(x))
+    a.W2, a.out2 = L.ptr(W2t), L.ptr(out2)
+    rc = int(L.lib().uvc_gemm_nt_lnbwd_proj(C.byref(a), L.cur_stream()))
+    if check:
+        L.check(rc, "uvc_gemm_nt_lnbwd_proj")
+    return rc
+
+
 def mlp_fused_fwd(x, gamma, beta, w1, b1, w2, b2, out, eps=1e-6, *, x_prev=None, gate=None, h=None, mean=None, rstd=None, gp=None, u=None,
                   next_gamma=None, next_beta=None, next_h=None, next_mean=None, next_rstd=None):
     _chk(x, gamma, beta, w1, b1, w2, b2, out, x_prev, gate, h, mean, rstd, gp, u, next_gamma, next_beta, next_h, next_mean, next_rstd)
```

Measured after the change: 47940 images/sec (median of 6 runs). No clear change (+0.4%).
